# alepnabil/fmcw_radar_processing

Measured on AMD Instinct MI355X. Metric: radar frames/sec (range-FFT+Doppler+STFT) + achieved HBM GB/s vs roofline, higher is better.
Workload: dtype f32

## Files before the change

### fmcw_radar_processing_amd/csrc/fmcw_api.cpp

```cpp
#include "api_internal.h"
#include "xcd_ctr_plan.h"

#include <dlfcn.h>

#include <cmath>
#include <cstdio>
#include <cstring>

namespace {
thread_local std::string g_err;
}

namespace fmcw {

int fail(int code, const std::string& msg) {
  g_err = msg;
  return code;
}

int set_error(int code, const char* msg) { return fail(code, msg); }

void par_memcpy(void* dst, const void* src, size_t n) {
  const unsigned hw = std::max(1u, std::thread::hardware_concurrency());
  const unsigned T = n >= (8u << 20) ? std::min(8u, hw) : 1u;
  if (T == 1) {
    std::memcpy(dst, src, n);
    return;
  }
  const size_t per = ((n + T - 1) / T + 4095) & ~(size_t)4095;
  std::vector<std::thread> th;
  for (unsigned t = 0; t < T; ++t) {
    const size_t o = (size_t)t * per;
    if (o >= n) break;
    th.emplace_back([=] { std::memcpy(static_cast<char*>(dst) + o, static_cast<const char*>(src) + o, std::min(per, n - o)); });
  }
  for (auto& x : th) x.join();
}

const Rccl& rccl() {
  static Rccl r = [] {
    Rccl x;
    void* h = nullptr;
    for (const char* name : {"librccl.so.1", "librccl.so", "/opt/rocm/lib/librccl.so.1"}) {
      h = dlopen(name, RTLD_NOW | RTLD_NOLOAD);
      if (h) break;
    }
    if (!h) h = dlopen("librccl.so.1", RTLD_NOW | RTLD_GLOBAL);
    if (!h) h = dlopen("/opt/rocm/lib/librccl.so.1", RTLD_NOW | RTLD_GLOBAL);
    if (!h) return x;
    x.comm_init_all = reinterpret_cast<decltype(x.comm_init_all)>(dlsym(h, "ncclCommInitAll"));
    x.comm_destroy = reinterpret_cast<decltype(x.comm_destroy)>(dlsym(h, "ncclCommDestroy"));
    x.all_reduce = reinterpret_cast<decltype(x.all_reduce)>(dlsym(h, "ncclAllReduce"));
    x.group_start = reinterpret_cast<decltype(x.group_start)>(dlsym(h, "ncclGroupStart"));
    x.group_end = reinterpret_cast<decltype(x.group_end)>(dlsym(h, "ncclGroupEnd"));
    x.error_string = reinterpret_cast<decltype(x.error_string)>(dlsym(h, "ncclGetErrorString"));
    x.ok = x.comm_init_all && x.comm_destroy && x.all_reduce && x.group_start && x.group_end && x.error_string;
    return x;
  }();
  return r;
}

}

fmcw_ctx::~fmcw_ctx() {
  for (ncclComm_t m : comms) (void)rccl().comm_destroy(m);
  for (fmcw_ctx* q : peers) delete q;
  (void)hipSetDevice(device);
  if (stream) (void)hipStreamSynchronize(stream);
  for (auto& pd : pending) { (void)hipEventDestroy(pd.a); (void)hipEventDestroy(pd.b); }
  for (auto e : pool) (void)hipEventDestroy(e);
  for (int i = 0; i < kSlots; ++i)
    for (hipEvent_t e : {ev_k1[i], ev_k2[i], ev_k3[i]})
      if (e) (void)hipEventDestroy(e);
  for (hipEvent_t e : {ev_fork, ev_join, ev_h2d[0], ev_h2d[1], ev_comp[0], ev_comp[1], ev_d2h[0], ev_d2h[1]})
    if (e) (void)hipEventDestroy(e);
  for (hipStream_t x : {sd, sx, cin, cout})
    if (x) { (void)hipStreamSynchronize(x); (void)hipStreamDestroy(x); }
  if (stream) (void)hipStreamDestroy(stream);
}

float2* fmcw_ctx::stft_tab(hipStream_t st, size_t bytes, int* status) {
  float2* t = static_cast<float2*>(s_tabs.get(st, bytes + STFT_TAPS_BYTES, status));
  if (t) {
    s_tabs.last->key = nullptr;
    s_tabs.last->key_n = 0;
  }
  return t;
}

float2* fmcw_ctx::stft_tab64(hipStream_t st, const float* d_win, int nfft, bool* build, int* status) {
  float2* t = static_cast<float2*>(s_tabs.get(st, (size_t)(nfft / 2 + 1) * 20 * 8 + STFT_TAPS_BYTES, status));
  if (!t) return nullptr;
  PerStream::Entry* e = s_tabs.last;
  *build = !(e->key == d_win && e->key_n == nfft);
  e->key = d_win;
  e->key_n = nfft;
  return t;
}

namespace {

int check_params(const fmcw_params* p) {
  if (!p) return fail(FMCW_E_ARG, "params is NULL");
  if (p->nts < 1 || p->nts > 65536) return fail(FMCW_E_ARG, "nts out of range [1, 65536]");
  if (p->pn < 1 || p->pn > 65536) return fail(FMCW_E_ARG, "pn out of range [1, 65536]");
  if (!fmcw::range_size_supported(p->nr)) return fail(FMCW_E_ARG, "nr must be a power of two in [16, 2048]");
  if (!fmcw::doppler_size_supported(p->nd)) return fail(FMCW_E_ARG, "nd must be a power of two in [2, 1024]");
  if (p->max_targets < 1 || p->max_targets > 8) return fail(FMCW_E_ARG, "max_targets must be in [1, 8]");
  if (!(p->dist_per_bin > 0.f)) return fail(FMCW_E_ARG, "dist_per_bin must be > 0");
  return FMCW_OK;
}

int build_calw(fmcw_ctx* c, float if_scale, hipStream_t s) {
  const size_t n = c->h_wr.size();
  std::vector<float> t(4 * n);
  for (size_t i = 0; i < n; ++i) {
    t[4 * i] = c->h_cal[2 * i];
    t[4 * i + 1] = c->h_cal[2 * i + 1];
    t[4 * i + 2] = (float)((double)if_scale * c->h_wr[i]);
    t[4 * i + 3] = c->h_wr[i];
  }
  CHK(c->calw.ensure(t.size() * 4));
  HIPCHK(hipMemcpyAsync(c->calw.p, t.data(), t.size() * 4, hipMemcpyHostToDevice, s));
  HIPCHK(hipStreamSynchronize(s));
  c->calw_scale = if_scale;
  return FMCW_OK;
}

int check_ctx(fmcw_ctx* c, const fmcw_params* p) {
  if (!c) return fail(FMCW_E_ARG, "ctx is NULL");
  CHK(check_params(p));
  if (!c->taps) return fail(FMCW_E_STATE, "fmcw_set_taps has not been called");
  if (p->nts != c->p.nts || p->pn != c->p.pn || p->nr != c->p.nr || p->nd != c->p.nd)
    return fail(FMCW_E_STATE, "nts/pn/nr/nd differ from the ones given to fmcw_set_taps");
  CHK(set_device(c));
  if (p->if_scale != c->calw_scale) {
    HIPCHK(hipDeviceSynchronize());
    CHK(build_calw(c, p->if_scale, c->stream));
  }
  return FMCW_OK;
}

int upload_twiddles(DevBuf& buf, int n, hipStream_t s) {
  std::vector<float> tw(2 * (size_t)n);
  for (int i = 0; i < n; ++i) {
    const double a = -2.0 * M_PI * (double)i / (double)n;
    tw[2 * i] = (float)std::cos(a);
    tw[2 * i + 1] = (float)std::sin(a);
  }
  CHK(buf.ensure(tw.size() * sizeof(float)));
  HIPCHK(hipMemcpyAsync(buf.p, tw.data(), tw.size() * sizeof(float), hipMemcpyHostToDevice, s));
  HIPCHK(hipStreamSynchronize(s));
  return FMCW_OK;
}

int64_t default_chunk(const fmcw_params* p) {
  const int64_t per_frame = (int64_t)p->pn * p->nr * 8;
  int64_t c = (256ll << 20) / std::max<int64_t>(per_frame, 1);
  return std::max<int64_t>(c, 1);
}

int range_cpt(int nr, int64_t nchirps) {
  const int T = nr >= 16 ? nr / 16 : 1;
  const int teams = T >= 256 ? 1 : 256 / T;
  const int64_t c = nchirps / ((int64_t)teams * 2048);
  return (int)std::max<int64_t>(1, std::min<int64_t>(8, c));
}


}

extern "C" {

int32_t fmcw_abi_version(void) { return FMCW_ABI_VERSION; }

const char* fmcw_last_error(void) { return g_err.c_str(); }

int fmcw_device_count(int32_t* n) {
  if (!n) return fail(FMCW_E_ARG, "n is NULL");
  int d = 0;
  hipError_t e = hipGetDeviceCount(&d);
  if (e != hipSuccess) {
    *n = 0;
    return fail(FMCW_E_HIP, std::string("hipGetDeviceCount: ") + hipGetErrorString(e));
  }
  *n = d;
  return FMCW_OK;
}

int fmcw_default_devices(int32_t cap, int32_t* ids, int32_t* n) {
  if (!ids || !n || cap < 1) return fail(FMCW_E_ARG, "ids/n NULL or cap < 1");
  *n = 0;
  const char* env = std::getenv("FMCW_DEVICES");
  std::string v = env ? env : "";
  v.erase(std::remove_if(v.begin(), v.end(), [](char ch) { return ch == ' ' || ch == '\t'; }), v.end());
  std::vector<long> want;
  if (!v.empty() && v != "all") {
    size_t pos = 0;
    while (pos <= v.size()) {
      const size_t end = std::min(v.find(',', pos), v.size());
      const std::string tok = v.substr(pos, end - pos);
      char* stop = nullptr;
      const long id = tok.empty() ? -1 : std::strtol(tok.c_str(), &stop, 10);
      if (tok.empty() || *stop != '\0' || id < 0) return fail(FMCW_E_ARG, "FMCW_DEVICES: malformed list '" + v + "'");
      want.push_back(id);
      pos = end + 1;
    }
    if ((int64_t)want.size() > cap) return fail(FMCW_E_ARG, "FMCW_DEVICES: more ids than cap");
  }
  int nd = 0;
  hipError_t e = hipGetDeviceCount(&nd);
  if (e != hipSuccess) return fail(FMCW_E_HIP, std::string("hipGetDeviceCount: ") + hipGetErrorString(e));
  if (want.empty()) {
    if (nd < 1) return fail(FMCW_E_HIP, "no HIP device present");
    const int m = std::min<int>(nd, cap);
    for (int i = 0; i < m; ++i) ids[i] = i;
    *n = m;
    return FMCW_OK;
  }
  for (size_t i = 0; i < want.size(); ++i) {
    if (want[i] >= nd)
      return fail(FMCW_E_ARG, "FMCW_DEVICES: device " + std::to_string(want[i]) + " not present (" +
                                  std::to_string(nd) + " devices)");
    ids[i] = (int32_t)want[i];
  }
  *n = (int32_t)want.size();
  return FMCW_OK;
}

static int ctx_create_one(int32_t device_id, fmcw_ctx** out) {
  *out = nullptr;
  int nd = 0;
  HIPCHK(hipGetDeviceCount(&nd));
  if (device_id < 0 || device_id >= nd)
    return fail(FMCW_E_HIP, "device " + std::to_string(device_id) + " not present (" + std::to_string(nd) + " devices)");
  HIPCHK(hipSetDevice(device_id));
  hipDeviceProp_t prop;
  HIPCHK(hipGetDeviceProperties(&prop, device_id));
  if (std::strncmp(prop.gcnArchName, "gfx950", 6) != 0)
    return fail(FMCW_E_HIP, std::string("libfmcw is built for gfx950, device is ") + prop.gcnArchName);
  auto* c = new fmcw_ctx();
  c->device = device_id;
  bool ok = hipStreamCreateWithFlags(&c->stream, hipStreamNonBlocking) == hipSuccess &&
            hipStreamCreateWithFlags(&c->sd, hipStreamNonBlocking) == hipSuccess &&
            hipStreamCreateWithFlags(&c->sx, hipStreamNonBlocking) == hipSuccess &&
            hipStreamCreateWithFlags(&c->cin, hipStreamNonBlocking) == hipSuccess &&
            hipStreamCreateWithFlags(&c->cout, hipStreamNonBlocking) == hipSuccess;
  for (int i = 0; i < 2; ++i)
    for (hipEvent_t* e : {&c->ev_h2d[i], &c->ev_comp[i], &c->ev_d2h[i]})
      ok = ok && hipEventCreateWithFlags(e, hipEventDisableTiming) == hipSuccess;
  for (int i = 0; i < fmcw_ctx::kSlots; ++i)
    for (hipEvent_t* e : {&c->ev_k1[i], &c->ev_k2[i], &c->ev_k3[i]})
      ok = ok && hipEventCreateWithFlags(e, hipEventDisableTiming | fmcw::kEvDevice) == hipSuccess;
  for (hipEvent_t* e : {&c->ev_fork, &c->ev_join})
    ok = ok && hipEventCreateWithFlags(e, hipEventDisableTiming | fmcw::kEvDevice) == hipSuccess;
  if (!ok) {
    delete c;
    return fail(FMCW_E_HIP, "stream/event creation failed");
  }
  *out = c;
  return FMCW_OK;
}

int fmcw_ctx_create(int32_t n_devices, const int32_t* device_ids, fmcw_ctx** out) {
  if (!out) return fail(FMCW_E_ARG, "out is NULL");
  *out = nullptr;
  if (n_devices < 1 || n_devices > 64) return fail(FMCW_E_ARG, "n_devices must be in [1, 64]");
  std::vector<int> ids(n_devices);
  for (int i = 0; i < n_devices; ++i) ids[i] = device_ids ? device_ids[i] : i;
  fmcw_ctx* c = nullptr;
  CHK(ctx_create_one(ids[0], &c));
  for (int i = 1; i < n_devices; ++i) {
    fmcw_ctx* q = nullptr;
    const int st = ctx_create_one(ids[i], &q);
    if (st != FMCW_OK) {
      delete c;
      return st;
    }
    c->peers.push_back(q);
  }
  std::vector<int> sorted = ids;
  std::sort(sorted.begin(), sorted.end());
  const bool distinct = std::adjacent_find(sorted.begin(), sorted.end()) == sorted.end();
  if (n_devices > 1 && distinct) {
    if (!rccl().ok) {
      delete c;
      return fail(FMCW_E_HIP, "RCCL (librccl.so.1) not found: needed for a context over several devices");
    }
    c->comms.assign(n_devices, nullptr);
    const ncclResult_t r = rccl().comm_init_all(c->comms.data(), n_devices, ids.data());
    if (r != ncclSuccess) {
      c->comms.clear();
      const std::string msg = std::string("ncclCommInitAll: ") + rccl().error_string(r);
      delete c;
      return fail(FMCW_E_HIP, msg);
    }
  }
  *out = c;
  return FMCW_OK;
}

int fmcw_ctx_devices(fmcw_ctx* c, int32_t* n_devices, int32_t* device_ids, int32_t* rccl_comms) {
  if (!c || !n_devices) return fail(FMCW_E_ARG, "NULL argument");
  *n_devices = 1 + (int32_t)c->peers.size();
  if (device_ids) {
    device_ids[0] = c->device;
    for (size_t i = 0; i < c->peers.size(); ++i) device_ids[i + 1] = c->peers[i]->device;
  }
  if (rccl_comms) *rccl_comms = c->comms.empty() ? 0 : 1;
  return FMCW_OK;
}

int fmcw_ctx_destroy(fmcw_ctx* c) {
  if (!c) return FMCW_OK;
  delete c;
  return FMCW_OK;
}

int fmcw_set_taps(fmcw_ctx* c, const fmcw_params* p, const float* range_win, const float* doppler_win,
                  const float* calib) {
  if (!c) return fail(FMCW_E_ARG, "ctx is NULL");
  CHK(check_params(p));
  if (!range_win || !doppler_win || !calib) return fail(FMCW_E_ARG, "taps pointer is NULL");
  CHK(set_device(c));
  hipStream_t s = c->stream;
  HIPCHK(hipDeviceSynchronize());
  CHK(c->wd.ensure((size_t)p->pn * 4));
  CHK(c->cal.ensure((size_t)p->nts * 8));
  HIPCHK(hipMemcpyAsync(c->wd.p, doppler_win, (size_t)p->pn * 4, hipMemcpyHostToDevice, s));
  HIPCHK(hipMemcpyAsync(c->cal.p, calib, (size_t)p->nts * 8, hipMemcpyHostToDevice, s));
  c->h_wr.assign(range_win, range_win + p->nts);
  c->h_cal.assign(calib, calib + 2 * (size_t)p->nts);
  double sr = 0, si = 0;
  for (int n = 0; n < p->nts; ++n) { sr += calib[2 * n]; si += calib[2 * n + 1]; }
  c->cal_sum = make_float2((float)sr, (float)si);
  CHK(build_calw(c, p->if_scale, s));
  CHK(upload_twiddles(c->tw_nr, p->nr, s));
  CHK(upload_twiddles(c->tw_nd, p->nd, s));
  c->p = *p;
  c->taps = true;
  c->x_tab_ok = false;
  HIPCHK(hipStreamSynchronize(s));
  for (fmcw_ctx* q : c->peers) CHK(fmcw_set_taps(q, p, range_win, doppler_win, calib));
  return FMCW_OK;
}

int fmcw_set_chunk_frames(fmcw_ctx* c, int64_t frames) {
  if (!c) return fail(FMCW_E_ARG, "ctx is NULL");
  if (frames < 0) return fail(FMCW_E_ARG, "frames < 0");
  c->chunk_frames = frames;
  for (fmcw_ctx* q : c->peers) q->chunk_frames = frames;
  return FMCW_OK;
}

int fmcw_set_pipeline(fmcw_ctx* c, int32_t mode) {
  if (!c) return fail(FMCW_E_ARG, "ctx is NULL");
  if (mode != FMCW_PIPE_AUTO && mode != FMCW_PIPE_STREAMS && mode != FMCW_PIPE_ONEPASS && mode != FMCW_PIPE_XCD)
    return fail(FMCW_E_ARG, "bad pipeline mode");
  c->pipe_mode = mode;
  for (fmcw_ctx* q : c->peers) q->pipe_mode = mode;
  return FMCW_OK;
}

static int xcd_check(fmcw_ctx* c) {
  if (!c->xcd_used) return FMCW_OK;
  unsigned e = 0;
  HIPCHK(hipMemcpy(&e, c->x_err.p, sizeof(e), hipMemcpyDeviceToHost));
  c->xcd_used = false;
  if (!e) return FMCW_OK;
  HIPCHK(hipMemset(c->x_err.p, 0, sizeof(e)));
  return fail(FMCW_E_HIP, (e & 2) ? "XCD schedule: an XCD received more than 32 workgroups (outputs invalid)"
                                  : "XCD schedule: a range-cube hand-off timed out (outputs invalid)");
}

int fmcw_rdx_clock(fmcw_ctx* c, double* mhz, double* us) {
  if (!c || !mhz) return fail(FMCW_E_ARG, "ctx / mhz is NULL");
  *mhz = 0.0;
  if (us) *us = 0.0;
  CHK(set_device(c));
  if (!c->x_clk.p) return FMCW_OK;
  unsigned long long h[4] = {};
  HIPCHK(hipStreamSynchronize(c->stream));
  HIPCHK(hipDeviceSynchronize());
  HIPCHK(hipMemcpy(h, c->x_clk.p, sizeof(h), hipMemcpyDeviceToHost));
  if (h[3] > h[1] && h[2] > h[0]) {
    *mhz = (double)(h[2] - h[0]) / (double)(h[3] - h[1]) * 100.0;
    if (us) *us = (double)(h[3] - h[1]) / 100.0;
  }
  return FMCW_OK;
}

int fmcw_copy_device(fmcw_ctx* c, const void* d_src, void* d_dst, int64_t bytes, void* stream) {
  if (!c) return fail(FMCW_E_ARG, "ctx is NULL");
  if (!d_src || !d_dst || bytes < 0) return fail(FMCW_E_ARG, "bad copy arguments");
  CHK(set_device(c));
  HIPCHK(fmcw::launch_copy16(d_src, d_dst, bytes, pick(c, stream)));
  return FMCW_OK;
}

int fmcw_synchronize(fmcw_ctx* c) {
  if (!c) return fail(FMCW_E_ARG, "ctx is NULL");
  CHK(set_device(c));
  HIPCHK(hipStreamSynchronize(c->stream));
  return xcd_check(c);
}

int fmcw_timing_enable(fmcw_ctx* c, int32_t enable) {
  if (!c) return fail(FMCW_E_ARG, "ctx is NULL");
  if (enable < 0 || enable > 3) return fail(FMCW_E_ARG, "timing level must be 0, 1, 2 or 3");
  c->timing = enable;
  return FMCW_OK;
}

static int timing_collect(fmcw_ctx* c) {
  for (auto& pd : c->pending) {
    HIPCHK(hipEventSynchronize(pd.b));
    float ms = 0.f;
    HIPCHK(hipEventElapsedTime(&ms, pd.a, pd.b));
    c->total_ms[pd.stage] += ms;
    c->launches[pd.stage] += 1;
    c->pool.push_back(pd.a);
    c->pool.push_back(pd.b);
  }
  c->pending.clear();
  return FMCW_OK;
}

int fmcw_timing_read(fmcw_ctx* c, int32_t stage, double* total_ms, int64_t* launches) {
  if (!c) return fail(FMCW_E_ARG, "ctx is NULL");
  if (stage < 0 || stage >= kStages) return fail(FMCW_E_ARG, "stage out of range");
  CHK(set_device(c));
  CHK(timing_collect(c));
  if (total_ms) *total_ms = c->total_ms[stage];
  if (launches) *launches = c->launches[stage];
  return FMCW_OK;
}

int fmcw_timing_reset(fmcw_ctx* c) {
  if (!c) return fail(FMCW_E_ARG, "ctx is NULL");
  CHK(set_device(c));
  CHK(timing_collect(c));
  for (int i = 0; i < kStages; ++i) { c->total_ms[i] = 0; c->launches[i] = 0; }
  return FMCW_OK;
}

static int build_xcd_tab(fmcw_ctx* c, hipStream_t s) {
  const int NR = c->p.nr;
  std::vector<double> cr(NR), ci(NR);
  for (int i = 0; i < NR; ++i) {
    const double a = -2.0 * M_PI * (double)i / (double)NR;
    cr[i] = std::cos(a);
    ci[i] = std::sin(a);
  }
  std::vector<float> xt(2 * (size_t)fmcw::XT_SIZE);
  auto xput = [&](int idx, int e1024) { xt[2 * idx] = (float)cr[e1024 & (NR - 1)]; xt[2 * idx + 1] = (float)ci[e1024 & (NR - 1)]; };
  for (int l = 0; l < 64; ++l) {
    for (int k1 = 1; k1 < 8; ++k1)
      for (int e = 0; e < 2; ++e) xput(fmcw::XT_R1 + (2 * (k1 - 1) + e) * 64 + l, (2 * l + e) * k1);
    for (int s1 = 1; s1 < 16; ++s1) xput(fmcw::XT_R2 + (s1 - 1) * 64 + l, 8 * ((l & 7) * s1));
    for (int d0 = 1; d0 < 16; ++d0) xput(fmcw::XT_D1 + (d0 - 1) * 64 + l, 4 * ((l & 15) * d0));
    for (int k1 = 1; k1 < 8; ++k1) xput(fmcw::XT_H1 + (k1 - 1) * 64 + l, 2 * l * k1);
    for (int s1 = 1; s1 < 8; ++s1) xput(fmcw::XT_H2 + (s1 - 1) * 64 + l, 16 * ((l & 7) * s1));
    for (int s2 = 0; s2 < 8; ++s2) xput(fmcw::XT_HC + s2 * 64 + l, l + 64 * s2);
  }
  CHK(c->x_tab.ensure(xt.size() * 4));
  HIPCHK(hipMemcpyAsync(c->x_tab.p, xt.data(), xt.size() * 4, hipMemcpyHostToDevice, s));
  HIPCHK(hipStreamSynchronize(s));
  c->x_tab_ok = true;
  return FMCW_OK;
}

static unsigned host_s16mask(const fmcw_params* p, int NR) {
  {
    const char* e = std::getenv("FMCW_S16");
    if (e && e[0] == '0') return 0u;
  }
  const double dpb = p->dist_per_bin;
  if (!(dpb > 0.0) || !std::isfinite(dpb) || !std::isfinite(p->min_d) || !std::isfinite(p->max_d)) return 0u;
  const double lo_d = std::floor((double)p->min_d / dpb) - 2, hi_d = std::ceil((double)p->max_d / dpb) + 2;
  const int lo = (int)std::max(0.0, std::min((double)NR, lo_d));
  const int hi = (int)std::max(-1.0, std::min((double)NR - 1, hi_d));
  unsigned m = 0;
  for (int b = 0; b < NR / 128; ++b)
    if (hi < lo || 128 * b + 127 < lo || 128 * b > hi) m |= 1u << b;
  return m;
}

struct SlowLeg {
  int32_t* list;
  int64_t* len;
  float* pmax;
};

static int process_onepass(fmcw_ctx* c, const fmcw_params* p, const void* d_iq, int h, int64_t F, float* d_prof,
                           int32_t* d_count, int32_t* d_ridx, float* d_rmag, int32_t* d_didx, float* d_slow,
                           void* d_rd, int64_t probe_column, float* d_probe, const SlowLeg* leg, hipStream_t s) {
  const int C = p->pn, S = p->nts, NR = p->nr, ND = p->nd, M = p->max_targets;
  const int64_t chunk = std::min<int64_t>(F, c->chunk_frames > 0 ? c->chunk_frames : 8192);
  const int tiles = fmcw::XCD_TILES, ncand = fmcw::XCD_CAND;
  const int TC = tiles * ncand;
  const int slots = fmcw::XCD_MAX_SLOTS;
  {
#ifdef FMCW_XCUBE_PAD_AB
    CHK(c->x_cube.ensure((size_t)8 * slots * fmcw::XCD_TILES * C * 32 * 8 + ((size_t)1 << 30)));
#else
    CHK(c->x_cube.ensure((size_t)8 * slots * fmcw::XCD_TILES * C * 32 * 8));
#endif
    if (!c->x_ctr.p) {
      CHK(c->x_ctr.ensure(sizeof(unsigned) * 2 * fmcw::XCD_CTR_WORDS));
      HIPCHK(hipMemsetAsync(c->x_ctr.p, 0, sizeof(unsigned) * 2 * fmcw::XCD_CTR_WORDS, s));
      c->x_ctr_set = 0;
    }
    if (!c->x_clk.p) {
      CHK(c->x_clk.ensure(4 * sizeof(unsigned long long)));
      HIPCHK(hipMemsetAsync(c->x_clk.p, 0, 4 * sizeof(unsigned long long), s));
    }
    if (!c->x_err.p) {
      CHK(c->x_err.ensure(sizeof(unsigned)));
      HIPCHK(hipMemsetAsync(c->x_err.p, 0, sizeof(unsigned), s));
    }
  }
  CHK(c->op_rowpk.ensure((size_t)chunk * NR * 8));
  CHK(c->op_cidx.ensure((size_t)chunk * TC * 4));
  CHK(c->op_crows.ensure((size_t)chunk * TC * C * 4));
  int32_t* det_done = nullptr;
  if (leg) {
    int st = FMCW_OK;
    bool fresh = false;
    det_done = static_cast<int32_t*>(c->det_done.get(s, 9 * 128, &st, &fresh));
    CHK(st);
    if (fresh) HIPCHK(hipMemsetAsync(det_done, 0, 9 * 128, s));
  }
  const int64_t pframe = probe_column > 0 ? (probe_column - 1) / C : -1;
  const int pchirp = probe_column > 0 ? (int)((probe_column - 1) % C) : 0;
  if (!c->x_tab_ok) CHK(build_xcd_tab(c, s));
  if (pframe >= 0 && d_probe) {
    fmcw::ProbeArgs pa{};
    pa.iq = d_iq; pa.h = h;
    pa.frame = pframe; pa.chirp = pchirp; pa.C = C; pa.S = S; pa.NR = NR;
    pa.calw = c->calw.as<float4>(); pa.tw_nr = c->tw_nr.as<float2>(); pa.probe_mag = d_probe;
    HIPCHK(fmcw::launch_probe(pa, s));
  }
  StageTimer span(c, 7, s, 1);
  for (int64_t f0 = 0; f0 < F; f0 += chunk) {
    const int64_t nf = std::min(chunk, F - f0);
    fmcw::OnePassArgs a{};
    a.iq = static_cast<const char*>(d_iq) + (size_t)f0 * C * S * (h ? 4 : 8);
    a.h = h;
    a.rd_scale = h ? 1.0f / ((float)NR * ND) : 1.0f;
    a.F = nf; a.C = C; a.S = S;
    a.calw = c->calw.as<float4>();
    a.tw_nr = c->tw_nr.as<float2>(); a.tw_nd = c->tw_nd.as<float2>(); a.wd = c->wd.as<float>();
    a.rd = d_rd ? static_cast<char*>(d_rd) + (size_t)f0 * NR * ND * (h ? 4 : 8) : nullptr;
    a.profile = d_prof + f0 * NR;
    a.rowpk = c->op_rowpk.as<int2>();
    a.cand_idx = c->op_cidx.as<int32_t>();
    a.cand_rows = c->op_crows.as<float>();
    a.range_thr = p->range_thr; a.min_d = p->min_d; a.max_d = p->max_d; a.dist_per_bin = p->dist_per_bin;
    const bool xmemset = [] { const char* e = std::getenv("FMCW_XCD_MEMSET"); return e && e[0] == '1'; }();
    const fmcw::XcdCtrPlan xp = fmcw::xcd_ctr_plan(c->x_ctr_set, xmemset);
    a.xcube = c->x_cube.as<float2>(); a.xerr = c->x_err.as<unsigned>();
    a.xctr = c->x_ctr.as<unsigned>() + xp.count_set * fmcw::XCD_CTR_WORDS;
    a.xclr = xp.clear_set < 0 ? nullptr : c->x_ctr.as<unsigned>() + xp.clear_set * fmcw::XCD_CTR_WORDS;
    a.xmemset = xp.memset_first ? 1 : 0;
#ifdef FMCW_XCUBE_PAD_AB
    if (const char* e = std::getenv("FMCW_XCUBE_PAD")) {
      const size_t pad = std::min<size_t>((size_t)std::strtoull(e, nullptr, 0), (size_t)1 << 30) & ~(size_t)255;
      a.xcube = reinterpret_cast<float2*>(c->x_cube.as<char>() + pad);
    }
#endif
    a.slots = slots; a.xtab = c->x_tab.as<float2>(); a.cal_sum = c->cal_sum;
    a.clk = c->x_clk.as<unsigned long long>();
    a.s16mask = h ? host_s16mask(p, NR) : 0u;
    a.nteams = c->xcd_teams > 0 ? c->xcd_teams : 0;
    std::memcpy(a.xcc_team, c->xcc_team, sizeof(a.xcc_team));
    {
      const char* e = std::getenv("FMCW_ONEPASS_FORCE_FIX");
      a.force_fix = (e && e[0] == '1') ? 1 : 0;
    }
#if defined(XK_STAMPS) || defined(XK_SKEW)
    static unsigned long long* xdbg = nullptr;
    if (!xdbg) HIPCHK(hipMalloc(&xdbg, (size_t)1 << 20));
    a.dbg = xdbg;
#endif
    {
      StageTimer tm(c, 8, s, 2);
      {
        HIPCHK(fmcw::launch_xcd(a, s));
        c->xcd_used = true;
        if (nf > 0) c->x_ctr_set = xp.next_set;
#ifdef XK_SKEW
        {
          constexpr int ST = 256;
          const int nblk = 32 * a.nteams;
          std::vector<unsigned long long> hh((size_t)nblk * 2 * ST);
          HIPCHK(hipStreamSynchronize(s));
          HIPCHK(hipMemcpy(hh.data(), a.dbg, hh.size() * 8, hipMemcpyDeviceToHost));
          double spread = 0, lag_min = 0, lag_max = 0, lag_mean = 0, pub_to_first_poll = 0;
          long n = 0;
          std::vector<long> last(32, 0), first(32, 0);
          for (int xx = 0; xx < a.nteams; ++xx)
            for (int j = 8; j < ST - 8; ++j) {
              unsigned long long pmin = ~0ull, pmax = 0, qmin = ~0ull, qmax = 0;
              double qs = 0;
              int kl = 0, kf = 0;
              for (int kk = 0; kk < 32; ++kk) {
                const unsigned long long p_ = hh[((size_t)(xx * 32 + kk)) * 2 * ST + 2 * j];
                const unsigned long long q_ = hh[((size_t)(xx * 32 + kk)) * 2 * ST + 2 * j + 1];
                if (p_ > pmax) { pmax = p_; kl = kk; }
                if (p_ < pmin) { pmin = p_; kf = kk; }
                qmin = std::min(qmin, q_); qmax = std::max(qmax, q_);
                qs += (double)q_;
              }
              if (!pmin || !qmin) continue;
              spread += (double)(pmax - pmin);
              lag_min += (double)qmin - (double)pmax;
              lag_max += (double)qmax - (double)pmax;
              lag_mean += qs / 32 - (double)pmax;
              pub_to_first_poll += (double)qmin - (double)pmin;
              ++last[kl]; ++first[kf]; ++n;
            }
          if (n) {
            std::fprintf(stderr, "xk-skew (us, %ld team-steps): publish spread %.2f | poll return after the last publish: "
                         "first %.2f mean %.2f last %.2f\n", n, spread / n / 100, lag_min / n / 100, lag_mean / n / 100,
                         lag_max / n / 100);
            std::fprintf(stderr, "xk-skew last publisher by member:");
            for (int kk = 0; kk < 32; ++kk) std::fprintf(stderr, " %ld", last[kk]);
            std::fprintf(stderr, "\nxk-skew first publisher by member:");
            for (int kk = 0; kk < 32; ++kk) std::fprintf(stderr, " %ld", first[kk]);
            std::fprintf(stderr, "\n");
          }
        }
#endif
#ifdef XK_STAMPS
        {
          const int nblk = 32 * a.nteams;
          std::vector<unsigned long long> hh(nblk * 32);
          HIPCHK(hipStreamSynchronize(s));
          HIPCHK(hipMemcpy(hh.data(), a.dbg, hh.size() * 8, hipMemcpyDeviceToHost));
          static const char* nm[10] = {"B1", "stage", "B2", "rows", "pubwait+B3", "cand", "R1+ld+D3",
                                       "poll+grp", "TD..R3", "RD"};
          for (int wv = 0; wv < 2; ++wv) {
            double ph[10] = {}, steps = 0;
            for (int bb = 0; bb < nblk; ++bb) {
              for (int q = 0; q < 10; ++q) ph[q] += (double)hh[(bb * 2 + wv) * 16 + q];
              steps += (double)hh[(bb * 2 + wv) * 16 + 15];
            }
            double tot = 0;
            std::fprintf(stderr, "xk-stamps wave %d (us/step):", wv * 4);
            for (int q = 0; q < 10; ++q) { std::fprintf(stderr, " %s %.2f |", nm[q], ph[q] / steps / 100); tot += ph[q]; }
            double cyc = 0, rt = 0;
            for (int bb = 0; bb < nblk; ++bb) { cyc += (double)hh[(bb * 2 + wv) * 16 + 13]; rt += (double)hh[(bb * 2 + wv) * 16 + 14]; }
            std::fprintf(stderr, " sum %.2f | clock %.3f GHz\n", tot / steps / 100, rt > 0 ? cyc / rt * 0.1 : 0.0);
          }
        }
#endif
      }
      tm.done();
    }
    fmcw::Detect1pArgs k{};
    k.profile = a.profile; k.rowpk = a.rowpk; k.rd = a.rd; k.ND = ND; k.rd_h = h; k.cand_idx = a.cand_idx; k.cand_rows = a.cand_rows;
    k.tiles = tiles; k.ncand = ncand;
    k.nframes = (int)nf; k.NR = NR; k.C = C; k.M = M;
    k.det.ND = ND; k.det.C = C; k.det.M = M;
    k.det.range_thr = p->range_thr; k.det.doppler_thr = p->doppler_thr;
    k.det.min_d = p->min_d; k.det.max_d = p->max_d; k.det.dist_per_bin = p->dist_per_bin;
    k.det.fallback = p->doppler_fallback_idx;
    k.det.cube_unscale = 1.0f; k.det.rd_unscale = 1.0f / a.rd_scale;
    k.count = d_count + f0; k.ridx = d_ridx + f0 * M; k.rmag = d_rmag + f0 * M; k.didx = d_didx + f0 * M;
    k.slow_mag = d_slow + f0 * C;
    k.iq = a.iq; k.h = h; k.S = S; k.calw = a.calw; k.tw_nr = a.tw_nr;
    if (leg && f0 + nf == F) {
      k.done = det_done; k.count_all = d_count; k.F_all = F; k.pn = C;
      k.list = leg->list; k.len = leg->len; k.pmax_reset = leg->pmax;
    }
    {
      StageTimer tm(c, 2, s, 2);
      HIPCHK(fmcw::launch_detect_1p(k, s));
      tm.done();
    }
  }
  if (leg) CHK(c->det_done.done(s));
  span.done();
  return FMCW_OK;
}

static int process_device_impl(fmcw_ctx* c, const fmcw_params* p, const void* d_iq, int32_t in_dtype, int64_t F,
                               float* d_prof, int32_t* d_count, int32_t* d_ridx, float* d_rmag, int32_t* d_didx,
                               float* d_slow, void* d_cube, void* d_rd, int32_t out_dtype, int64_t probe_column,
                               float* d_probe, const SlowLeg* leg, void* stream) {
  CHK(check_ctx(c, p));
  if (F < 0) return fail(FMCW_E_ARG, "F < 0");
  if (F == 0) return FMCW_OK;
  if (in_dtype != FMCW_C64 && in_dtype != FMCW_C32H) return fail(FMCW_E_ARG, "bad in_dtype");
  if (out_dtype != FMCW_C64 && out_dtype != FMCW_C32H) return fail(FMCW_E_ARG, "bad out_dtype");
  if (!d_iq || !d_prof || !d_count || !d_ridx || !d_rmag || !d_didx || !d_slow)
    return fail(FMCW_E_ARG, "required device pointer is NULL");
  const int S = p->nts, C = p->pn, NR = p->nr, ND = p->nd, M = p->max_targets;
  if (probe_column < 0 || probe_column > F * (int64_t)C) return fail(FMCW_E_ARG, "probe_column out of range");
  hipStream_t s = pick(c, stream);
  const bool onepass_ok = !d_cube && (!d_rd || out_dtype == in_dtype) && fmcw::onepass_supported(S, C, NR, ND);
  const bool want = c->pipe_mode == FMCW_PIPE_ONEPASS || c->pipe_mode == FMCW_PIPE_XCD;
  if (want || (c->pipe_mode == FMCW_PIPE_AUTO && onepass_ok)) {
    if (!onepass_ok)
      return fail(FMCW_E_ARG, "single-pass schedule: needs nr 1024, pn == nd == 256, even nts <= nr, "
                              "the RD map in the IQ dtype and no range cube");
    if (c->xcd_teams < 0) {
      int n = 0;
      HIPCHK(fmcw::xcd_census(&n, c->xcc_team));
      const char* e = std::getenv("FMCW_NO_XCD");
      c->xcd_teams = (e && e[0] == '1') ? 0 : n;
    }
    if (c->xcd_teams > 0)
      return process_onepass(c, p, d_iq, in_dtype == FMCW_C32H ? 1 : 0, F, d_prof, d_count, d_ridx, d_rmag, d_didx,
                             d_slow, d_rd, probe_column, d_probe, leg, s);
    if (want)
      return fail(FMCW_E_ARG, "XCD schedule: needs 32 CUs per XCD and a grid of one workgroup per CU dealt 32 per XCD");
  }
  const int64_t chunk = c->chunk_frames > 0 ? c->chunk_frames : default_chunk(p);
  const int cube_dt = d_cube ? out_dtype : FMCW_C64;
  const int rd_dt = d_rd ? out_dtype : FMCW_C64;
  const float cube_scale = cube_dt == FMCW_C32H ? 1.0f / NR : 1.0f;
  const float rd_scale = rd_dt == FMCW_C32H ? 1.0f / ((float)NR * ND) : 1.0f;
  const int64_t cf = std::min(chunk, F);
  const size_t cube_slot = (size_t)cf * C * NR * 8, rd_slot = (size_t)cf * NR * ND * 8;
  constexpr int NS = fmcw_ctx::kSlots;
  if (!d_cube) CHK(c->scratch_cube.ensure(NS * cube_slot));
  if (!d_rd) CHK(c->scratch_rd.ensure(NS * rd_slot));
  const int64_t pframe = probe_column > 0 ? (probe_column - 1) / C : -1;
  const int pchirp = probe_column > 0 ? (int)((probe_column - 1) % C) : 0;
  hipStream_t sd = c->sd, sx = c->sx;
  if (F <= chunk) sd = sx = s;
  if (const char* e = std::getenv("FMCW_ONE_STREAM"); e && e[0] == '1') sd = sx = s;
  const bool split = sd != s || sx != s;
  StageTimer span(c, 7, s, 1);
  if (split) {
    HIPCHK(hipEventRecord(c->ev_fork, s));
    HIPCHK(hipStreamWaitEvent(sd, c->ev_fork, 0));
    HIPCHK(hipStreamWaitEvent(sx, c->ev_fork, 0));
  }

  int64_t i = 0;
  for (int64_t f0 = 0; f0 < F; f0 += chunk, ++i) {
    const int b = (int)(i % NS);
    const int64_t nf = std::min(chunk, F - f0);
    if (split && i >= NS) HIPCHK(hipStreamWaitEvent(s, c->ev_k3[b], 0));
    char* cube = d_cube ? static_cast<char*>(d_cube) + (size_t)f0 * C * NR * esize(cube_dt)
                        : c->scratch_cube.as<char>() + b * cube_slot;
    char* rd = d_rd ? static_cast<char*>(d_rd) + (size_t)f0 * NR * ND * esize(rd_dt)
                    : c->scratch_rd.as<char>() + b * rd_slot;

    fmcw::RangeArgs ra{};
    ra.iq = static_cast<const char*>(d_iq) + (size_t)f0 * C * S * esize(in_dtype);
    ra.in_dtype = in_dtype;
    ra.nchirps = nf * C;
    ra.C = C; ra.S = S; ra.NR = NR;
    ra.calw = c->calw.as<float4>();
    ra.cal_sum = c->cal_sum;
    ra.if_scale = p->if_scale;
    ra.tw = c->tw_nr.as<float2>();
    ra.cube = cube;
    ra.cube_dtype = cube_dt;
    ra.cube_scale = cube_scale;
    ra.profile = nullptr;
    ra.cpt = range_cpt(NR, ra.nchirps);
    {
      StageTimer tm(c, 0, s, 2);
      HIPCHK(fmcw::launch_range(ra, s));
      tm.done();
    }
    if (split) {
      HIPCHK(hipEventRecord(c->ev_k1[b], s));
      HIPCHK(hipStreamWaitEvent(sd, c->ev_k1[b], 0));
    }

    fmcw::DopplerArgs da{};
    da.cube = cube; da.cube_dtype = cube_dt;
    da.cube_unscale = 1.0f / cube_scale; da.rd_scale = rd_scale;
    da.nframes = (int)nf; da.C = C; da.NR = NR; da.ND = ND;
    da.wd = c->wd.as<float>();
    da.tw = c->tw_nd.as<float2>();
    da.rd = rd; da.rd_dtype = rd_dt;
    da.profile = d_prof + f0 * NR;
    {
      StageTimer tm(c, 1, sd, 2);
      HIPCHK(fmcw::launch_doppler(da, sd));
      tm.done();
    }
    if (split) {
      HIPCHK(hipEventRecord(c->ev_k2[b], sd));
      HIPCHK(hipStreamWaitEvent(sx, c->ev_k2[b], 0));
    }

    fmcw::DetectArgs ka{};
    ka.profile = d_prof + f0 * NR;
    ka.rd = rd; ka.rd_dtype = rd_dt;
    ka.cube = cube; ka.cube_dtype = cube_dt;
    ka.cube_unscale = 1.0f / cube_scale; ka.rd_unscale = 1.0f / rd_scale;
    ka.nframes = (int)nf; ka.NR = NR; ka.ND = ND; ka.C = C; ka.M = M;
    ka.range_thr = p->range_thr; ka.doppler_thr = p->doppler_thr;
    ka.min_d = p->min_d; ka.max_d = p->max_d; ka.dist_per_bin = p->dist_per_bin;
    ka.fallback = p->doppler_fallback_idx;
    ka.count = d_count + f0;
    ka.ridx = d_ridx + f0 * M;
    ka.rmag = d_rmag + f0 * M;
    ka.didx = d_didx + f0 * M;
    ka.slow_mag = d_slow + f0 * C;
    ka.probe_frame = (pframe >= f0 && pframe < f0 + nf) ? pframe - f0 : -1;
    ka.probe_chirp = pchirp;
    ka.probe_mag = d_probe;
    {
      StageTimer tm(c, 2, sx, 2);
      HIPCHK(fmcw::launch_detect(ka, sx));
      tm.done();
    }
    if (split) HIPCHK(hipEventRecord(c->ev_k3[b], sx));
  }
  span.s = sd;
  span.done();
  if (split) {
    HIPCHK(hipEventRecord(c->ev_join, sx));
    HIPCHK(hipStreamWaitEvent(s, c->ev_join, 0));
  }
  if (leg) {
    HIPCHK(fmcw::launch_compact(d_count, F, C, leg->list, leg->len, s));
    if (leg->pmax) HIPCHK(hipMemsetAsync(leg->pmax, 0, 4, s));
  }
  return FMCW_OK;
}

int fmcw_process_device(fmcw_ctx* c, const fmcw_params* p, const void* d_iq, int32_t in_dtype, int64_t F,
                        float* d_prof, int32_t* d_count, int32_t* d_ridx, float* d_rmag, int32_t* d_didx,
                        float* d_slow, void* d_cube, void* d_rd, int32_t out_dtype, int64_t probe_column,
                        float* d_probe, void* stream) {
  return process_device_impl(c, p, d_iq, in_dtype, F, d_prof, d_count, d_ridx, d_rmag, d_didx, d_slow, d_cube, d_rd,
                             out_dtype, probe_column, d_probe, nullptr, stream);
}

int fmcw_process_slow_device(fmcw_ctx* c, const fmcw_params* p, const void* d_iq, int32_t in_dtype, int64_t F,
                             float* d_prof, int32_t* d_count, int32_t* d_ridx, float* d_rmag, int32_t* d_didx,
                             float* d_slow, void* d_rd, int32_t out_dtype, int32_t* d_frame_list, int64_t* d_len,
                             float* d_pmax, void* stream) {
  if (!d_frame_list || !d_len) return fail(FMCW_E_ARG, "d_frame_list / d_len is NULL");
  if (F == 0 && c) {
    CHK(check_ctx(c, p));
    hipStream_t s = pick(c, stream);
    HIPCHK(hipMemsetAsync(d_len, 0, 8, s));
    if (d_pmax) HIPCHK(hipMemsetAsync(d_pmax, 0, 4, s));
    return FMCW_OK;
  }
  const SlowLeg leg{d_frame_list, d_len, d_pmax};
  return process_device_impl(c, p, d_iq, in_dtype, F, d_prof, d_count, d_ridx, d_rmag, d_didx, d_slow, nullptr, d_rd,
                             out_dtype, 0, nullptr, &leg, stream);
}

int fmcw_range_fft_device(fmcw_ctx* c, const fmcw_params* p, const void* d_iq, int32_t in_dtype, int64_t F,
                          void* d_cube, int32_t out_dtype, float* d_prof, void* stream) {
  CHK(check_ctx(c, p));
  if (F < 0) return fail(FMCW_E_ARG, "F < 0");
  if (F == 0) return FMCW_OK;
  if (!d_iq || !d_cube || !d_prof) return fail(FMCW_E_ARG, "required device pointer is NULL");
  if (in_dtype != FMCW_C64 && in_dtype != FMCW_C32H) return fail(FMCW_E_ARG, "bad in_dtype");
  if (out_dtype != FMCW_C64 && out_dtype != FMCW_C32H) return fail(FMCW_E_ARG, "bad out_dtype");
  hipStream_t s = pick(c, stream);
  HIPCHK(hipMemsetAsync(d_prof, 0, (size_t)F * p->nr * 4, s));
  fmcw::RangeArgs ra{};
  ra.iq = d_iq; ra.in_dtype = in_dtype;
  ra.nchirps = F * p->pn;
  ra.C = p->pn; ra.S = p->nts; ra.NR = p->nr;
  ra.calw = c->calw.as<float4>(); ra.cal_sum = c->cal_sum; ra.if_scale = p->if_scale;
  ra.tw = c->tw_nr.as<float2>();
  ra.cube = d_cube; ra.cube_dtype = out_dtype;
  ra.cube_scale = out_dtype == FMCW_C32H ? 1.0f / p->nr : 1.0f;
  ra.profile = d_prof;
  int cpt = 8;
  if (const char* e = std::getenv("FMCW_K1_CPT")) cpt = std::max(1, std::min(64, std::atoi(e)));
  while (cpt > 1 && (p->pn % cpt) != 0) cpt >>= 1;
  ra.cpt = cpt;
  const int T = p->nr >= 16 ? p->nr / 16 : 1;
  const int teams = T >= 256 ? 1 : 256 / T;
  const int64_t per_wg = (int64_t)teams * cpt;
  ra.parts = (per_wg < p->pn && p->pn % per_wg == 0) ? (int)(p->pn / per_wg) : 0;
  if (ra.parts > 1) {
    int st = FMCW_OK;
    ra.prof_part = static_cast<float*>(c->k1_part.get(s, (size_t)F * ra.parts * p->nr * 4, &st));
    CHK(st);
  }
  StageTimer tm(c, 6, s);
  HIPCHK(fmcw::launch_range(ra, s));
  if (ra.parts > 1) {
    HIPCHK(fmcw::launch_profile_reduce(ra.prof_part, ra.parts, F, p->nr, d_prof, s));
    CHK(c->k1_part.done(s));
  }
  tm.done();
  return FMCW_OK;
}

int fmcw_compact_device(fmcw_ctx* c, const int32_t* d_count, int64_t F, int32_t pn, int32_t* d_list,
                        int64_t* d_len, void* stream) {
  if (!c) return fail(FMCW_E_ARG, "ctx is NULL");
  if (F < 0 || pn < 1) return fail(FMCW_E_ARG, "bad F / pn");
  if (!d_count || !d_list || !d_len) return fail(FMCW_E_ARG, "NULL device pointer");
  CHK(set_device(c));
  hipStream_t s = pick(c, stream);
  StageTimer tm(c, 3, s);
  HIPCHK(fmcw::launch_compact(d_count, F, pn, d_list, d_len, s));
  tm.done();
  return FMCW_OK;
}

}

struct BigOut {
  char* host;
  size_t fbytes;
};
template <typename Run>
static int host_pipeline(fmcw_ctx* c, const void* iq, int64_t F, size_t fin, const BigOut (&big)[2], Run&& run) {
  hipStream_t s = c->stream;
  const int64_t Fc = host_chunk(fin, F);
  const size_t slot_in = (size_t)Fc * fin;
  size_t slot_big[2], off_big[2] = {0, 0}, slot_out = 0;
  bool any = false;
  for (int q = 0; q < 2; ++q) {
    slot_big[q] = big[q].host ? (size_t)Fc * big[q].fbytes : 0;
    off_big[q] = slot_out;
    slot_out += slot_big[q];
    any = any || big[q].host;
  }
  CHK(c->h_iq.ensure(2 * slot_in));
  CHK(c->pin_in.ensure(2 * slot_in));
  if (any) {
    CHK(c->h_rd.ensure(2 * slot_out));
    CHK(c->pin_out.ensure(2 * slot_out));
  }
  const int64_t n = (F + Fc - 1) / Fc;
  auto drain = [&](int64_t j) -> int {
    const int b = (int)(j & 1);
    const int64_t f0 = j * Fc, nf = std::min(Fc, F - f0);
    HIPCHK(hipEventSynchronize(c->ev_d2h[b]));
    for (int q = 0; q < 2; ++q)
      if (big[q].host)
        par_memcpy(big[q].host + (size_t)f0 * big[q].fbytes, c->pin_out.at(b * slot_out + off_big[q]),
                   (size_t)nf * big[q].fbytes);
    return FMCW_OK;
  };
  const bool single = n == 1;
  hipStream_t cin = single ? s : c->cin;
  if (!single) {
    HIPCHK(hipEventRecord(c->ev_fork, s));
    HIPCHK(hipStreamWaitEvent(c->cin, c->ev_fork, 0));
  }
  for (int64_t i = 0; i < n; ++i) {
    const int b = (int)(i & 1);
    const int64_t f0 = i * Fc, nf = std::min(Fc, F - f0);
    if (i >= 2) HIPCHK(hipEventSynchronize(c->ev_h2d[b]));
    par_memcpy(c->pin_in.at(b * slot_in), static_cast<const char*>(iq) + (size_t)f0 * fin, (size_t)nf * fin);
    if (i >= 2) HIPCHK(hipStreamWaitEvent(c->cin, c->ev_comp[b], 0));
    HIPCHK(hipMemcpyAsync(c->h_iq.as<char>() + b * slot_in, c->pin_in.at(b * slot_in), (size_t)nf * fin,
                          hipMemcpyHostToDevice, cin));
    if (!single) {
      HIPCHK(hipEventRecord(c->ev_h2d[b], c->cin));
      HIPCHK(hipStreamWaitEvent(s, c->ev_h2d[b], 0));
    }
    if (any && i >= 2) {
      HIPCHK(hipStreamWaitEvent(s, c->ev_d2h[b], 0));
      CHK(drain(i - 2));
    }
    char* d_big[2];
    for (int q = 0; q < 2; ++q) d_big[q] = big[q].host ? c->h_rd.as<char>() + b * slot_out + off_big[q] : nullptr;
    CHK(run(c->h_iq.as<char>() + b * slot_in, f0, nf, d_big));
    HIPCHK(hipEventRecord(c->ev_comp[b], s));
    if (any) {
      HIPCHK(hipStreamWaitEvent(c->cout, c->ev_comp[b], 0));
      for (int q = 0; q < 2; ++q)
        if (big[q].host)
          HIPCHK(hipMemcpyAsync(c->pin_out.at(b * slot_out + off_big[q]), d_big[q], (size_t)nf * big[q].fbytes,
                                hipMemcpyDeviceToHost, c->cout));
      HIPCHK(hipEventRecord(c->ev_d2h[b], c->cout));
    }
  }
  if (any)
    for (int64_t j = std::max<int64_t>(0, n - 2); j < n; ++j) CHK(drain(j));
  return FMCW_OK;
}

extern "C" {

static int process_host_one(fmcw_ctx* c, const fmcw_params* p, const void* iq, int32_t in_dtype, int64_t F,
                            float* prof, int32_t* count, int32_t* ridx, float* rmag, int32_t* didx, float* slow,
                            float* cube, float* rd, int64_t probe_column, float* probe) {
  CHK(check_ctx(c, p));
  if (F < 0) return fail(FMCW_E_ARG, "F < 0");
  if (F == 0) return FMCW_OK;
  if (!iq || !prof || !count || !ridx || !rmag || !didx || !slow) return fail(FMCW_E_ARG, "required pointer is NULL");
  if (in_dtype != FMCW_C64 && in_dtype != FMCW_C32H) return fail(FMCW_E_ARG, "bad in_dtype");
  const int S = p->nts, C = p->pn, NR = p->nr, ND = p->nd, M = p->max_targets;
  hipStream_t s = c->stream;
  Arena ar;
  const size_t o_prof = ar.add((size_t)F * NR * 4), o_count = ar.add((size_t)F * 4), o_ridx = ar.add((size_t)F * M * 4),
               o_rmag = ar.add((size_t)F * M * 4), o_didx = ar.add((size_t)F * M * 4), o_slow = ar.add((size_t)F * C * 4),
               o_probe = ar.add(probe ? (size_t)NR * 4 : 0);
  CHK(c->h_small.ensure(ar.off));
  CHK(c->pin_small.ensure(ar.off));
  char* const hs = c->h_small.as<char>();
  auto at = [&](size_t o) { return reinterpret_cast<float*>(hs + o); };
  auto ati = [&](size_t o) { return reinterpret_cast<int32_t*>(hs + o); };
  const size_t fin = (size_t)C * S * esize(in_dtype);
  const BigOut big[2] = {{reinterpret_cast<char*>(cube), (size_t)C * NR * 8}, {reinterpret_cast<char*>(rd), (size_t)NR * ND * 8}};
  CHK(host_pipeline(c, iq, F, fin, big, [&](char* d_in, int64_t f0, int64_t nf, char* const* d_big) {
    const int64_t pc = probe && probe_column > f0 * C && probe_column <= (f0 + nf) * C ? probe_column - f0 * C : 0;
    return fmcw_process_device(c, p, d_in, in_dtype, nf, at(o_prof) + f0 * NR, ati(o_count) + f0, ati(o_ridx) + f0 * M,
                               at(o_rmag) + f0 * M, ati(o_didx) + f0 * M, at(o_slow) + f0 * C, d_big[0], d_big[1], FMCW_C64,
                               pc, pc ? at(o_probe) : nullptr, s);
  }));
  HIPCHK(hipMemcpyAsync(c->pin_small.p, hs, ar.off, hipMemcpyDeviceToHost, s));
  HIPCHK(hipStreamSynchronize(s));
  HIPCHK(hipStreamSynchronize(c->cout));
  const char* ps = c->pin_small.at(0);
  par_memcpy(prof, ps + o_prof, (size_t)F * NR * 4);
  std::memcpy(count, ps + o_count, (size_t)F * 4);
  std::memcpy(ridx, ps + o_ridx, (size_t)F * M * 4);
  std::memcpy(rmag, ps + o_rmag, (size_t)F * M * 4);
  std::memcpy(didx, ps + o_didx, (size_t)F * M * 4);
  par_memcpy(slow, ps + o_slow, (size_t)F * C * 4);
  if (probe) std::memcpy(probe, ps + o_probe, (size_t)NR * 4);
  return xcd_check(c);
}

static int range_fft_host_one(fmcw_ctx* c, const fmcw_params* p, const void* iq, int32_t in_dtype, int64_t F,
                              float* cube, float* prof) {
  CHK(check_ctx(c, p));
  if (F < 0) return fail(FMCW_E_ARG, "F < 0");
  if (F == 0) return FMCW_OK;
  if (!iq || !cube || !prof) return fail(FMCW_E_ARG, "required pointer is NULL");
  if (in_dtype != FMCW_C64 && in_dtype != FMCW_C32H) return fail(FMCW_E_ARG, "bad in_dtype");
  const int S = p->nts, C = p->pn, NR = p->nr;
  hipStream_t s = c->stream;
  CHK(c->h_prof.ensure((size_t)F * NR * 4));
  const BigOut big[2] = {{reinterpret_cast<char*>(cube), (size_t)C * NR * 8}, {nullptr, 0}};
  CHK(host_pipeline(c, iq, F, (size_t)C * S * esize(in_dtype), big, [&](char* d_in, int64_t f0, int64_t nf, char* const* d_big) {
    return fmcw_range_fft_device(c, p, d_in, in_dtype, nf, d_big[0], FMCW_C64, c->h_prof.as<float>() + f0 * NR, s);
  }));
  HIPCHK(hipMemcpyAsync(prof, c->h_prof.p, (size_t)F * NR * 4, hipMemcpyDeviceToHost, s));
  HIPCHK(hipStreamSynchronize(s));
  HIPCHK(hipStreamSynchronize(c->cout));
  return FMCW_OK;
}

}

extern "C" {

int fmcw_process(fmcw_ctx* c, const fmcw_params* p, const void* iq, int32_t in_dtype, int64_t F, float* prof,
                 int32_t* count, int32_t* ridx, float* rmag, int32_t* didx, float* slow, float* cube, float* rd,
                 int64_t probe_column, float* probe) {
  CHK(check_ctx(c, p));
  if (F < 0) return fail(FMCW_E_ARG, "F < 0");
  if (in_dtype != FMCW_C64 && in_dtype != FMCW_C32H) return fail(FMCW_E_ARG, "bad in_dtype");
  if (probe_column < 0 || probe_column > F * (int64_t)p->pn) return fail(FMCW_E_ARG, "probe_column out of range");
  const int C = p->pn, S = p->nts, NR = p->nr, ND = p->nd, M = p->max_targets;
  const size_t fin = (size_t)C * S * esize(in_dtype);
  return over_devices(c, F, [&](fmcw_ctx* d, int, int64_t f0, int64_t n) {
    const int64_t pc = probe_column > f0 * C && probe_column <= (f0 + n) * C ? probe_column - f0 * C : 0;
    return process_host_one(d, p, static_cast<const char*>(iq) + f0 * fin, in_dtype, n, prof + f0 * NR, count + f0,
                            ridx + f0 * M, rmag + f0 * M, didx + f0 * M, slow + f0 * C,
                            cube ? cube + f0 * (size_t)C * NR * 2 : nullptr, rd ? rd + f0 * (size_t)NR * ND * 2 : nullptr,
                            pc, pc ? probe : nullptr);
  });
}

int fmcw_range_fft(fmcw_ctx* c, const fmcw_params* p, const void* iq, int32_t in_dtype, int64_t F, float* cube,
                   float* prof) {
  CHK(check_ctx(c, p));
  if (F < 0) return fail(FMCW_E_ARG, "F < 0");
  if (in_dtype != FMCW_C64 && in_dtype != FMCW_C32H) return fail(FMCW_E_ARG, "bad in_dtype");
  const size_t fin = (size_t)p->pn * p->nts * esize(in_dtype);
  return over_devices(c, F, [&](fmcw_ctx* d, int, int64_t f0, int64_t n) {
    return range_fft_host_one(d, p, static_cast<const char*>(iq) + f0 * fin, in_dtype, n,
                              cube + f0 * (size_t)p->pn * p->nr * 2, prof + f0 * p->nr);
  });
}

int fmcw_synth_device(fmcw_ctx* c, const fmcw_params* p, int64_t frame0, int64_t F, void* d_iq, int32_t dtype,
                      void* stream) {
  CHK(check_ctx(c, p));
  if (F < 0 || frame0 < 0) return fail(FMCW_E_ARG, "F / frame0 < 0");
  if (!d_iq) return fail(FMCW_E_ARG, "d_iq is NULL");
  if (dtype != FMCW_C64 && dtype != FMCW_C32H) return fail(FMCW_E_ARG, "bad dtype");
  fmcw::SynthArgs a{};
  a.iq = d_iq; a.dtype = dtype; a.frame0 = frame0; a.nframes = F;
  a.C = p->pn; a.S = p->nts; a.NR = p->nr; a.ND = p->nd;
  a.dist_per_bin = p->dist_per_bin;
  a.cal = c->cal.as<float2>();
  HIPCHK(fmcw::launch_synth(a, pick(c, stream)));
  return FMCW_OK;
}

}
```

### fmcw_radar_processing_amd/csrc/fmcw_internal.h

```cpp
#pragma once
#include <hip/hip_runtime.h>
#include <stdint.h>

namespace fmcw {

#ifndef FMCW_EV_SYSFENCE
constexpr unsigned kEvDevice = hipEventDisableSystemFence;
#else
constexpr unsigned kEvDevice = 0;
#endif

struct RangeArgs {
  const void* iq;
  int in_dtype;
  int64_t nchirps;
  int C, S, NR;
  const float4* calw;
  float2 cal_sum;
  float if_scale;
  const float2* tw;
  void* cube;
  int cube_dtype;
  float cube_scale;
  float* profile;
  int cpt;
  float* prof_part;
  int parts;
};

struct DopplerArgs {
  const void* cube;
  int cube_dtype;
  float cube_unscale;
  float rd_scale;
  int nframes, C, NR, ND;
  const float* wd;
  const float2* tw;
  void* rd;
  int rd_dtype;
  float* profile;
};

struct DetectArgs {
  const float* profile;
  const void* rd;
  int rd_dtype;
  const void* cube;
  int cube_dtype;
  float cube_unscale, rd_unscale;
  int nframes, NR, ND, C, M;
  float range_thr, doppler_thr, min_d, max_d, dist_per_bin;
  int fallback;
  int32_t* count;
  int32_t* ridx;
  float* rmag;
  int32_t* didx;
  float* slow_mag;
  int64_t probe_frame;
  int probe_chirp;
  float* probe_mag;
};

struct DetectParams {
  int ND, C, M;
  float range_thr, doppler_thr, min_d, max_d, dist_per_bin;
  int fallback;
  float cube_unscale, rd_unscale;
};

struct OnePassArgs {
  const void* iq;
  int h;
  float rd_scale;
  int64_t F;
  int C, S;
  const float4* calw;
  const float2* tw_nr;
  const float2* tw_nd;
  const float* wd;
  void* rd;
  float* profile;
  int2* rowpk;
  int32_t* cand_idx;
  float* cand_rows;
  float range_thr, min_d, max_d, dist_per_bin;
  int force_fix;
  unsigned long long* dbg;
  unsigned long long* clk;
  float2* xcube;
  unsigned* xctr;
  unsigned* xclr;
  unsigned* xerr;
  int slots;
  unsigned s16mask;
  int nteams;
  int xmemset;
  int8_t xcc_team[16];
  const float2* xtab;
  float2 cal_sum;
};

constexpr int XCD_TILES = 32;
constexpr int XCD_CAND = 2;
constexpr int XCD_MAX_SLOTS = 4;
constexpr int XCD_GRID = 256;
constexpr int XCD_TICKETS = 8 * 2 * 32 * XCD_MAX_SLOTS;
constexpr int XCD_ABORT = XCD_TICKETS + 8 * 32;
constexpr int XCD_IDLE = XCD_ABORT + 32;
constexpr int XCD_CTR_WORDS = XCD_IDLE + 256 * 32;
constexpr int XT_R1 = 0;
constexpr int XT_R2 = 14 * 64;
constexpr int XT_D1 = 29 * 64;
constexpr int XT_H1 = 44 * 64;
constexpr int XT_H2 = 51 * 64;
constexpr int XT_HC = 58 * 64;
constexpr int XT_SIZE = 66 * 64;
#ifndef XK_HALF
__host__ __device__ inline int xcd_bin(int g, int p) {
  return (p >> 3) + 4 * (g & 1) + 8 * ((g >> 1) & 1) + 16 * (p & 7) + 128 * (g >> 2);
}
__host__ __device__ inline int xcd_group(int r) { return ((r >> 2) & 1) | (((r >> 3) & 1) << 1) | ((r >> 7) << 2); }
__host__ __device__ inline int xcd_pos(int r) { return ((r & 3) << 3) | ((r >> 4) & 7); }
#else
__host__ __device__ inline int xcd_bin(int g, int p) { return 32 * g + p; }
__host__ __device__ inline int xcd_group(int r) { return r >> 5; }
__host__ __device__ inline int xcd_pos(int r) { return r & 31; }
#endif

struct Detect1pArgs {
  const float* profile;
  const int2* rowpk;
  const void* rd;
  int ND, rd_h;
  const int32_t* cand_idx;
  const float* cand_rows;
  int tiles, ncand;
  int nframes, NR, C, M;
  DetectParams det;
  int32_t* count;
  int32_t* ridx;
  float* rmag;
  int32_t* didx;
  float* slow_mag;
  const void* iq;
  int h, S;
  const float4* calw;
  const float2* tw_nr;
  int32_t* done;
  const int32_t* count_all;
  int64_t F_all;
  int pn;
  int32_t* list;
  int64_t* len;
  float* pmax_reset;
};

hipError_t launch_detect_1p(const Detect1pArgs& a, hipStream_t s);
hipError_t launch_xcd(const OnePassArgs& a, hipStream_t s);
hipError_t xcd_census(int* nteams, int8_t* xcc_team);

struct ProbeArgs {
  const void* iq;
  int h;
  int64_t frame;
  int chirp, C, S, NR;
  const float4* calw;
  const float2* tw_nr;
  float* probe_mag;
};
hipError_t launch_probe(const ProbeArgs& a, hipStream_t s);
bool onepass_supported(int nts, int pn, int nr, int nd);

struct StftArgs {
  const float* slow_mag;
  const int32_t* frame_list;
  const int64_t* len;
  int pn;
  const float* halo;
  int n_halo;
  const int64_t* halo_len;
  const float* win;
  int wlen, hop, nfft;
  float inv_fs;
  int64_t max_seg;
  float* P;
  float* pmax;
  int64_t* nseg_out;
  const int32_t* bins;
  int ncol;
  const int32_t* tiles;
  int ntiles;
  int table_form;
};

bool stft_fast_path(int wlen, int hop);
bool stft64_form(int nfft);
enum StftForm { STFT_FORM_TABLE = 0, STFT_FORM_64F = 1, STFT_FORM_64M = 2 };
StftForm stft_form(const StftArgs& a, int mode, const float* dst);
hipError_t launch_stft_table(const float* win, int nfft, float2* tab, hipStream_t s);
hipError_t launch_stft20(const StftArgs& a, const float2* tab, int mode, float* dst, hipStream_t s, int64_t dst_cap,
                         int64_t tab_cap);


struct StftDbArgs {
  const float* P;
  const int64_t* nseg;
  int64_t max_seg;
  int nbins_in;
  const float* pmax;
  int nlog;
  const int32_t* lidx;
  const float* lw;
  float* out;
};

struct SynthArgs {
  void* iq;
  int dtype;
  int64_t frame0, nframes;
  int C, S, NR, ND;
  float dist_per_bin;
  const float2* cal;
};

hipError_t launch_range(const RangeArgs& a, hipStream_t s);
hipError_t launch_profile_reduce(const float* part, int parts, int64_t frames, int nr, float* profile, hipStream_t s);
hipError_t launch_doppler(const DopplerArgs& a, hipStream_t s);
hipError_t launch_detect(const DetectArgs& a, hipStream_t s);
hipError_t launch_compact(const int32_t* count, int64_t F, int pn, int32_t* frame_list, int64_t* len,
                          hipStream_t s);
hipError_t launch_stft_power(const StftArgs& a, hipStream_t s);
hipError_t launch_stft_db(const StftDbArgs& a, hipStream_t s);
hipError_t launch_synth(const SynthArgs& a, hipStream_t s);
hipError_t launch_fill_u32(uint32_t* p, uint32_t v, int64_t n, hipStream_t s);
hipError_t launch_copy16(const void* src, void* dst, int64_t bytes, hipStream_t s);


struct CfarArgs {
  const void* rd;
  int h;
  float scale;
  int64_t F;
  int NR, ND;
  int gr, gd, tr, td;
  int g0, g1;
  int K, local_max;
  float alpha;
  int RS, strips;
  int TC, tiles, waves;
  int32_t* sub_count;
  float4* sub_list;
  int32_t* det_count;
  int32_t* det_ridx;
  int32_t* det_didx;
  float* det_power;
  float* det_noise;
  uint8_t* mask;
};
void cfar_plan(CfarArgs& a, int64_t F);
size_t cfar_scratch_per_frame(const CfarArgs& a);
hipError_t launch_cfar(const CfarArgs& a, hipStream_t s);

struct SigArgs {
  const void* rd;
  int h;
  float scale2;
  int64_t F;
  int NR, ND;
  int g0, g1;
  int th;
  int dc;
  const int32_t* center;
  int64_t cstride;
  int SR, slabs;
  float* part;
  float* dt;
  float* rt;
  float* dt_max;
  float* rt_max;
};
void sig_plan(SigArgs& a);
size_t sig_scratch_per_frame(const SigArgs& a);
hipError_t launch_sig(const SigArgs& a, hipStream_t s);
hipError_t launch_sig_db(const float* map, int64_t n, const float* mx, float floor_db, float* out, hipStream_t s);

struct ClusterArgs {
  int64_t F;
  int ND;
  int K;
  int link_r, link_d, min_cells, max_tgt;
  const int32_t* det_count;
  const int32_t* det_ridx;
  const int32_t* det_didx;
  const float* det_power;
  const float* det_noise;
  int32_t* tgt_count;
  int32_t* cells; int32_t* pk_ridx; int32_t* pk_didx; int32_t* ext_r; int32_t* ext_d;
  float* pk_power; float* pk_noise; float* power; float* range; float* doppler;
  int32_t* det_label;
};
hipError_t launch_cluster(const ClusterArgs& a, hipStream_t s);

constexpr int kAoaChan = 8;
struct AoaArgs {
  int64_t F;
  int NR, ND;
  int K;
  int A;
  int M;
  int h;
  int tgt_any;
  float scale2;
  float kinv;
  float w[2 * kAoaChan];
  const void* rd[kAoaChan];
  const int32_t* det_count;
  const int32_t* det_ridx;
  const int32_t* det_didx;
  const int32_t* det_label;
  float* det_zre; float* det_zim; float* det_phase; float* det_sin;
  float* tgt_zre; float* tgt_zim; float* tgt_e0; float* tgt_e1; float* tgt_phase; float* tgt_sin; float* tgt_coh;
  int32_t* tgt_cells;
};
hipError_t launch_aoa(const AoaArgs& a, hipStream_t s);

constexpr int kTrackFields = 9;
constexpr int kTrackMax = 64;
constexpr int track_state_words(int max_trk) { return (kTrackFields * max_trk + 1 + 3) & ~3; }
struct TrackArgs {
  int64_t S, F;
  int NR, ND;
  int M, T;
  float wr, wd;
  float alpha_r, alpha_d, beta_r;
  int confirm_hits, max_coast;
  const int32_t* tgt_count;
  const float* range;
  const float* doppler;
  const float* power;
  uint32_t* state;
  int32_t* trk_count;
  int32_t* trk_id; int32_t* trk_status; int32_t* trk_age; int32_t* trk_misses;
  float* trk_range; float* trk_rate; float* trk_doppler; float* trk_power;
  int32_t* tgt_track;
};
hipError_t launch_track(const TrackArgs& a, hipStream_t s);

constexpr int kMtiRingC64 = 4;
constexpr int kMtiRingC32H = 8;
struct MtiArgs {
  const void* rd;
  void* out;
  float* bg;
  int32_t* seen;
  int64_t S, F;
  int64_t n16;
  int bpf;
  int h;
  int ring;
  float lambda;
  int ramp, freeze;
};
bool mti_ring_ok(int ring);
hipError_t launch_mti(const MtiArgs& a, hipStream_t s);

bool range_size_supported(int nr);
bool doppler_size_supported(int nd);

struct RenderArgs {
  const float* Q;
  int nq;
  const int64_t* nseg;
  const float* pmax;
  int nb, nfft, seam;
  double fs, t0, dt;
  double fmax, cmin, cmax;
  int W, H;
  uint8_t* img;
};
hipError_t launch_render(const RenderArgs& a, hipStream_t s);

}

#include "host_io.h"
```

### fmcw_radar_processing_amd/csrc/kernels_xcd.hip

```cpp
#include "op_math.h"

#include <cstdio>
#include <cstdlib>
#include <mutex>

namespace fmcw {
namespace xk {
using namespace op;

#ifdef XK_NOREF
#define XK_REF 0
#else
#define XK_REF 1
#endif
#ifndef XK_RD_AUX
#define XK_RD_AUX 2
#endif
constexpr int kRdAux = XK_RD_AUX;
#ifndef XK_LAG
#define XK_LAG 1
#endif
#ifndef XK_NS
#define XK_NS (2 * XK_LAG)
#endif
constexpr int kLag = XK_LAG;
#ifndef XK_POLLAT
#define XK_POLLAT 2
#endif
#ifndef XK_SKEW_STEPS
#define XK_SKEW_STEPS 256
#endif
static_assert(kLag == 1 || kLag == 2, "poll lag 1 (shipped) or 2");
constexpr int kNS = XK_NS;
static_assert(kNS >= 2 * kLag && kNS <= 4, "slot reuse: seeing ready(j - lag) proves frame j - 2 lag read");
constexpr int NK = 32;
constexpr int C = 256;
constexpr int NW = 8;
constexpr int GP = 32;
typedef unsigned u2v __attribute__((ext_vector_type(2)));
typedef unsigned u4v __attribute__((ext_vector_type(4)));
static_assert(NK * NW == C && NK * GP == NR && NK == XCD_TILES, "team geometry");

struct LdsX {
  union {
    f4v stg[C * 17];
    c2 rt[NW][1216];
  } u;
#ifndef XK_HALF
  f4v tw1[7][64];
  f4v tw2[8][64];
#else
  c2 th1[7][64];
  c2 th2[7][64];
  c2 thc[8][64];
#endif
  f4v twd[8][64];
  f4v wdl[4][64];
  f4v wq[4][64];
  c2 cwq[16][64];
  float key[GP];
#ifndef XK_NOREF
#ifndef XK_HALF
  f4v x0[512];
#else
  f4v x0[2][512];
  c2 psum[8];
#endif
#endif
};

__device__ __forceinline__ unsigned ld_flag(const unsigned* p) {
  const unsigned long long u = reinterpret_cast<unsigned long long>(p);
  const unsigned long long su = ((unsigned long long)__builtin_amdgcn_readfirstlane((unsigned)(u >> 32)) << 32) |
                                (unsigned)__builtin_amdgcn_readfirstlane((unsigned)u);
  unsigned v;
  asm volatile("s_load_dword %0, %1, 0x0 glc\n\ts_waitcnt lgkmcnt(0)" : "=s"(v) : "s"(reinterpret_cast<const unsigned*>(su)) : "memory");
  return v;
}
__device__ __forceinline__ void wait_ge(const unsigned* p, unsigned v, unsigned* abort, unsigned* err) {
  for (int it = 0; it < (1 << 20); ++it) {
    if (ld_flag(p) >= v) return;
    if ((it & 63) == 63 && ld_flag(abort)) return;
#ifndef XK_PSLEEP
#define XK_PSLEEP 2
#endif
    __builtin_amdgcn_s_sleep(XK_PSLEEP);
  }
  if (threadIdx.x == 0) {
    typedef __attribute__((address_space(1))) unsigned gu32;
    __hip_atomic_fetch_or((gu32*)abort, 1u, __ATOMIC_RELAXED, __HIP_MEMORY_SCOPE_AGENT);
    __hip_atomic_fetch_or((gu32*)err, 1u, __ATOMIC_RELAXED, __HIP_MEMORY_SCOPE_AGENT);
  }
}
__device__ __forceinline__ void cfence() { asm volatile("" ::: "memory"); }
__device__ __forceinline__ float2 h2f(unsigned b) {
  __half2 h;
  __builtin_memcpy(&h, &b, 4);
  return __half22float2(h);
}

template <int N> __device__ __forceinline__ void vm_wait() {
  static_assert(N >= 0 && N < 64, "vmcnt is 6 bits");
  asm volatile("s_waitcnt vmcnt(%0)" ::"n"(N) : "memory");
}


__device__ __forceinline__ float row_sum16(float v) {
  v += dppf<0xB1>(v);
  v += dppf<0x4E>(v);
  v += dppf<0x141>(v);
  return v + dppf<0x140>(v);
}
__device__ __forceinline__ int row_max16(int v) {
  v = max(v, dppi<0xB1>(v));
  v = max(v, dppi<0x4E>(v));
  v = max(v, dppi<0x141>(v));
  return max(v, dppi<0x140>(v));
}
__device__ __forceinline__ int row_min16(int v) {
  v = min(v, dppi<0xB1>(v));
  v = min(v, dppi<0x4E>(v));
  v = min(v, dppi<0x141>(v));
  return min(v, dppi<0x140>(v));
}

__device__ __forceinline__ f4v pair_cols(c2 A, c2 B, bool odd) {
  const c2 snd = odd ? A : B;
  const c2 rcv = c2{dppf<0xB1>(snd.x), dppf<0xB1>(snd.y)};
  return odd ? f4v{rcv.x, rcv.y, B.x, B.y} : f4v{A.x, A.y, rcv.x, rcv.y};
}

}

template <bool FULL, bool H, bool RD>
__global__ __launch_bounds__(512, 1) void k_rdx(OnePassArgs a) {
  using namespace xk;
  __shared__ __attribute__((aligned(16))) LdsX L;
  const int tid = threadIdx.x, lane = tid & 63;
  const int w = __builtin_amdgcn_readfirstlane(tid >> 6);
  __shared__ int team[2];
  __shared__ unsigned gflag;
  if (tid == 0) {
    gflag = 0;
    unsigned xcc;
    asm volatile("s_getreg_b32 %0, hwreg(HW_REG_XCC_ID)" : "=s"(xcc));
    const int xx = a.xcc_team[xcc & 15];
    int kk = NK;
    if (xx >= 0) kk = (int)__hip_atomic_fetch_add(a.xctr + XCD_TICKETS + xx * 32, 1u, __ATOMIC_RELAXED, __HIP_MEMORY_SCOPE_AGENT);
    if (kk >= NK) { atomicOr(a.xerr, 2u); atomicOr(a.xctr + XCD_ABORT, 1u); }
    team[0] = xx;
    team[1] = kk;
  }
  __syncthreads();
  if (a.xclr && blockIdx.x == 0)
    for (int i = tid; i < XCD_IDLE; i += 512) a.xclr[i] = 0u;
  const int x = __builtin_amdgcn_readfirstlane(team[0]), k = __builtin_amdgcn_readfirstlane(team[1]);
  if (k >= NK) return;
  const bool stamper = a.clk != nullptr && x == 0 && k == 0 && tid == 0;
  if (stamper) {
    a.clk[0] = __builtin_amdgcn_s_memtime();
    a.clk[1] = __builtin_amdgcn_s_memrealtime();
  }
  const int T = a.nteams;
  const int nj = a.F > x ? (int)((a.F - x + T - 1) / T) : 0;
  const int S = FULL ? NR : a.S, S2 = S >> 1, NS = a.slots;
  unsigned* ready = a.xctr + (x * 2 + 0) * 32 * XCD_MAX_SLOTS;
  auto rdy = [&](int s_) __attribute__((always_inline)) -> unsigned* { return &ready[s_ * 32]; };
#ifdef XK_DONE
  unsigned* done = ready + 32 * XCD_MAX_SLOTS;
#endif

  using TP = std::conditional_t<H, h4v, f4v>;
  const TP* __restrict__ iq = reinterpret_cast<const TP*>(a.iq);
  constexpr int kES = 8;
  constexpr int64_t kSlotBytes = (int64_t)NK * C * GP * kES;
  const unsigned s16m = H ? a.s16mask : 0u;
  const bool g16 = (s16m >> (k >> 2)) & 1;
  constexpr float kXS = 1.0f / NR, kXU = (float)NR;
#ifndef XK_NOREF
  TP x0n{};
  auto ld_ref = [&](int64_t f) __attribute__((always_inline)) {
    const TP* __restrict__ q = iq + f * C * (int64_t)S2;
    if constexpr (FULL) x0n = __builtin_nontemporal_load(q + tid);
    else x0n = __builtin_nontemporal_load(q + (tid < S2 ? tid : 0));
  };
  auto put_ref = [&](int b) __attribute__((always_inline)) {
    f4v t;
    if constexpr (H) t = __builtin_convertvector(x0n, f4v);
    else t = x0n;
    if constexpr (!FULL)
      if (tid >= S2) t = f4v{0.f, 0.f, 0.f, 0.f};
#ifndef XK_HALF
    (void)b;
    L.x0[tid] = t;
#else
    L.x0[b][tid] = t;
#endif
  };
  if (nj > 0) ld_ref(x);
#endif
#ifndef XK_HALF
  for (int i = tid; i < 44 * 64; i += 512) {
    const c2 v = tov(a.xtab[i]);
    const int l = i & 63;
    c2* d;
    if (i < XT_R2) { const int t = i >> 6; d = reinterpret_cast<c2*>(&L.tw1[t >> 1][l]) + (t & 1); }
    else if (i < XT_D1) { const int t = (i - XT_R2) >> 6; d = reinterpret_cast<c2*>(&L.tw2[t >> 1][l]) + (t & 1); }
    else { const int t = (i - XT_D1) >> 6; d = reinterpret_cast<c2*>(&L.twd[t >> 1][l]) + (t & 1); }
    *d = v;
  }
#else
  for (int i = XT_D1 + tid; i < XT_H1; i += 512) {
    const int t = (i - XT_D1) >> 6;
    reinterpret_cast<c2*>(&L.twd[t >> 1][i & 63])[t & 1] = tov(a.xtab[i]);
  }
  for (int i = tid; i < 22 * 64; i += 512) {
    const c2 v = tov(a.xtab[XT_H1 + i]);
    const int t = i >> 6, l = i & 63;
    if (t < 7) L.th1[t][l] = v;
    else if (t < 14) L.th2[t - 7][l] = v;
    else L.thc[t - 14][l] = v;
  }
#endif
  const float wd_scale = (H && RD ? a.rd_scale : 1.0f) * (g16 ? kXU : 1.0f);
  for (int i = tid; i < 16 * 64; i += 512)
    reinterpret_cast<float*>(&L.wdl[i >> 8][i & 63])[(i >> 6) & 3] = a.wd[(i & 15) + 16 * (i >> 6)] * wd_scale;
  for (int i = tid; i < 16 * 64; i += 512) {
    const int l = i & 63, v = i >> 6, n = 2 * l + (v & 1) + 128 * (v >> 1);
    const float4 cv = n < S ? a.calw[n] : make_float4(0.f, 0.f, 0.f, 0.f);
    reinterpret_cast<float*>(&L.wq[v >> 2][l])[v & 3] = cv.z;
    L.cwq[v][l] = c2{cv.x * cv.z, cv.y * cv.z};
  }
  const c2 csum = c2{a.cal_sum.x, a.cal_sum.y};
  const float invS = 1.0f / (float)S;
#ifndef XK_NOREF
  if (nj > 0) put_ref(0);
#endif
  __syncthreads();
#ifdef XK_PRIO
  if (w >= 4) __builtin_amdgcn_s_setprio(1);
#endif
#ifdef XK_STAMPS
  constexpr int NST = 10;
  unsigned long long st_acc[NST] = {}, st_t = __builtin_amdgcn_s_memrealtime();
  const unsigned long long st_c0 = __builtin_amdgcn_s_memtime(), st_r0 = st_t;
  auto stamp = [&](int i) {
    const unsigned long long n = __builtin_amdgcn_s_memrealtime();
    st_acc[i] += n - st_t;
    st_t = n;
  };
#else
  auto stamp = [](int) {};
#endif


  auto ld_chirp = [&](int64_t f, TP (&xin)[8]) __attribute__((always_inline)) {
    const TP* __restrict__ q = iq + (f * C + (k * NW + w)) * (int64_t)S2;
#pragma unroll
    for (int i = 0; i < 8; ++i) {
      const int p = lane + 64 * i;
      if constexpr (FULL) xin[i] = __builtin_nontemporal_load(q + p);
      else xin[i] = __builtin_nontemporal_load(q + (p < S2 ? p : 0));
    }
  };

  c2* const rt = L.u.rt[w];
#ifndef XK_HALF
#ifndef XK_NOREF
  const bool refw = k == 0 && w == 0;
  const float dsc = refw ? 0.f : 1.f;
  const c2 csum_w = refw ? csum : c2{0.f, 0.f};
#endif
  auto r_prep = [&](const TP (&xin)[8], c2 (&z0)[8], c2 (&z1)[8]) __attribute__((always_inline)) {
    c2 v[16];
#pragma unroll
    for (int i = 0; i < 8; ++i) {
      f4v t;
      if constexpr (H) t = __builtin_convertvector(xin[i], f4v);
      else t = xin[i];
#ifndef XK_NOREF
      t = __builtin_elementwise_fma(f4v{-dsc, -dsc, -dsc, -dsc}, L.x0[lane + 64 * i], t);
#endif
      if constexpr (!FULL)
        if (!(lane + 64 * i < S2)) t = f4v{0.f, 0.f, 0.f, 0.f};
      v[2 * i] = t.xy;
      v[2 * i + 1] = t.zw;
    }
    c2 sm = (v[0] + v[1]) + (v[2] + v[3]);
#pragma unroll
    for (int n = 4; n < 16; n += 4) sm += (v[n] + v[n + 1]) + (v[n + 2] + v[n + 3]);
    float wv[16];
#pragma unroll
    for (int g = 0; g < 4; ++g) {
      const f4v t = L.wq[g][lane];
      wv[4 * g] = t.x; wv[4 * g + 1] = t.y; wv[4 * g + 2] = t.z; wv[4 * g + 3] = t.w;
    }
#ifndef XK_NOREF
    const c2 mu = (wave_sum_c(sm) - csum_w) * invS;
    if (refw) {
#pragma unroll
      for (int n = 0; n < 16; ++n) v[n] = __builtin_elementwise_fma(v[n] - mu, c2{wv[n], wv[n]}, -L.cwq[n][lane]);
    } else {
#pragma unroll
      for (int n = 0; n < 16; ++n) v[n] = (v[n] - mu) * wv[n];
    }
#else
    const c2 mu = (wave_sum_c(sm) - csum) * invS;
#pragma unroll
    for (int n = 0; n < 16; ++n) v[n] = __builtin_elementwise_fma(v[n] - mu, c2{wv[n], wv[n]}, -L.cwq[n][lane]);
#endif
#pragma unroll
    for (int i = 0; i < 8; ++i) { z0[i] = v[2 * i]; z1[i] = v[2 * i + 1]; }
#ifndef XK_NORANGEFFT
    dft8p(z0);
    dft8p(z1);
#pragma unroll
    for (int k1 = 1; k1 < 8; ++k1) {
      const f4v t = L.tw1[k1 - 1][lane];
      z0[k1] = cmul_a(z0[k1], t.xy);
      z1[k1] = cmul_a(z1[k1], t.zw);
    }
#endif
  };
  const int k1 = lane >> 3, a0 = lane & 7, hh = lane & 7;
  auto r_mid = [&](c2 (&u)[16]) __attribute__((always_inline)) {
#ifndef XK_NORANGEFFT
    dft16p<1>(u);
#pragma unroll
    for (int s1 = 1; s1 < 16; s1 += 2) {
      const f4v t = L.tw2[s1 >> 1][lane];
      u[s1] = cmul_a(u[s1], t.xy);
      if (s1 < 15) u[s1 + 1] = cmul_a(u[s1 + 1], t.zw);
    }
#endif
  };
  auto r_t2 = [&](const c2 (&u)[16], c2 (&q0)[8], c2 (&q1)[8]) __attribute__((always_inline)) {
#pragma unroll
    for (int h = 0; h < 8; ++h)
      *reinterpret_cast<f4v*>(&rt[lane * 18 + 2 * h]) = f4v{u[2 * h].x, u[2 * h].y, u[2 * h + 1].x, u[2 * h + 1].y};
    cfence();
#pragma unroll
    for (int jj = 0; jj < 8; ++jj) {
      const f4v t = *reinterpret_cast<const f4v*>(&rt[(k1 * 8 + jj) * 18 + 2 * hh]);
      q0[jj] = t.xy;
      q1[jj] = t.zw;
    }
    cfence();
  };
  auto r_end = [&](c2 (&q0)[8], c2 (&q1)[8], char* __restrict__ slot) __attribute__((always_inline)) {
#ifndef XK_NORANGEFFT
    dft8p(q0);
    dft8p(q1);
#endif
    const int c = k * NW + w;
    const __amdgpu_buffer_rsrc_t rs = __builtin_amdgcn_make_buffer_rsrc(slot, (short)0, kSlotBytes, 0x00020000);
    const bool odd = lane & 1;
    const int gl = (lane >> 5) + (odd ? 2 : 0), el = c * GP + (lane & 31) - (odd ? 1 : 0);
#pragma unroll
    for (int s2 = 0; s2 < 8; ++s2) {
      const f4v v = pair_cols(q0[s2], q1[s2], odd);
      const int gb = (4 * s2 + gl) * C * GP * 8;
      if (H && ((s16m >> s2) & 1)) {
        const __half2 h0 = __floats2half2_rn(v.x * kXS, v.y * kXS), h1 = __floats2half2_rn(v.z * kXS, v.w * kXS);
        __builtin_amdgcn_raw_buffer_store_b64(u2v{__builtin_bit_cast(unsigned, h0), __builtin_bit_cast(unsigned, h1)}, rs,
                                              gb + el * 4, 0, 0);
      } else {
        __builtin_amdgcn_raw_buffer_store_b128(v, rs, gb + el * 8, 0, 0);
      }
    }
  };

#else
#ifdef XK_NOREF
#error "the half-frame build keeps the reference chirp"
#endif
  const int eh = w >> 2;
  const bool refw0 = k == 0 && (w & 3) == 0;
  typedef _Float16 h2v __attribute__((ext_vector_type(2)));
  using XH = std::conditional_t<H, h2v, c2>;
  auto ld_chirp_h = [&](int64_t f, int hf, XH (&xin)[8]) __attribute__((always_inline)) {
    const XH* __restrict__ q = reinterpret_cast<const XH*>(iq + (f * C + (128 * hf + 4 * k + (w & 3))) * (int64_t)S2) + eh;
#pragma unroll
    for (int i = 0; i < 8; ++i) {
      const int p = lane + 64 * i;
      if constexpr (FULL) xin[i] = __builtin_nontemporal_load(q + 2 * p);
      else xin[i] = __builtin_nontemporal_load(q + 2 * (p < S2 ? p : 0));
    }
  };
  auto rh_sum = [&](const XH (&xin)[8], bool refw, int xb, c2 (&d)[8]) __attribute__((always_inline)) {
    const float dsc = refw ? 0.f : 1.f;
    const c2* x0p = reinterpret_cast<const c2*>(L.x0[xb]) + eh;
    c2 sm{0.f, 0.f};
#pragma unroll
    for (int i = 0; i < 8; ++i) {
      c2 t;
      if constexpr (H) t = __builtin_convertvector(xin[i], c2);
      else t = xin[i];
      t = __builtin_elementwise_fma(c2{-dsc, -dsc}, x0p[2 * (lane + 64 * i)], t);
      if constexpr (!FULL)
        if (!(lane + 64 * i < S2)) t = c2{0.f, 0.f};
      d[i] = t;
      sm += t;
    }
    sm = wave_sum_c(sm);
    if (lane == 0) L.psum[w] = sm;
  };
  auto rh_prep = [&](c2 (&z)[8], bool refw) __attribute__((always_inline)) {
    const c2 csum_w = refw ? csum : c2{0.f, 0.f};
    const c2 mu = (L.psum[w] + L.psum[w ^ 4] - csum_w) * invS;
    float wv[8];
#pragma unroll
    for (int g = 0; g < 4; ++g) {
      const f4v t = L.wq[g][lane];
      wv[2 * g] = eh ? t.y : t.x;
      wv[2 * g + 1] = eh ? t.w : t.z;
    }
    if (refw) {
#pragma unroll
      for (int i = 0; i < 8; ++i) z[i] = __builtin_elementwise_fma(z[i] - mu, c2{wv[i], wv[i]}, -L.cwq[2 * i + eh][lane]);
    } else {
#pragma unroll
      for (int i = 0; i < 8; ++i) z[i] = (z[i] - mu) * wv[i];
    }
    dft8p(z);
#pragma unroll
    for (int k1 = 1; k1 < 8; ++k1) z[k1] = cmul_a(z[k1], L.th1[k1 - 1][lane]);
  };
  auto rh_t1w = [&](const c2 (&z)[8]) __attribute__((always_inline)) {
#pragma unroll
    for (int k1 = 0; k1 < 8; ++k1) rt[k1 * 72 + lane] = z[k1];
    cfence();
  };
  auto rh_t1r = [&](c2 (&u)[8]) __attribute__((always_inline)) {
#pragma unroll
    for (int l1 = 0; l1 < 8; ++l1) u[l1] = rt[(lane >> 3) * 72 + (lane & 7) + 8 * l1];
    cfence();
  };
  auto rh_mid = [&](c2 (&u)[8], c2 (&v)[8]) __attribute__((always_inline)) {
    dft8p(u);
#pragma unroll
    for (int s1 = 1; s1 < 8; ++s1) u[s1] = cmul_a(u[s1], L.th2[s1 - 1][lane]);
#pragma unroll
    for (int s1 = 0; s1 < 8; ++s1) rt[s1 * 97 + lane + 4 * (lane >> 5)] = u[s1];
    cfence();
    const int rb = (lane >> 3) * 97 + 8 * (lane & 7) + 4 * ((lane & 7) >> 2);
#pragma unroll
    for (int l0 = 0; l0 < 8; ++l0) v[l0] = rt[rb + l0];
    cfence();
    dft8p(v);
#pragma unroll
    for (int s2 = 0; s2 < 8; ++s2) rt[s2 * 64 + lane] = v[s2];
  };
  auto rh_end = [&](c2 (&v)[8], char* __restrict__ slot) __attribute__((always_inline)) {
    const c2* pr = L.u.rt[w ^ 4];
    if (eh) {
#pragma unroll
      for (int s2 = 0; s2 < 8; ++s2) v[s2] = pr[s2 * 64 + lane] - cmul_a(v[s2], L.thc[s2][lane]);
    } else {
#pragma unroll
      for (int s2 = 0; s2 < 8; ++s2) v[s2] = v[s2] + cmul_a(pr[s2 * 64 + lane], L.thc[s2][lane]);
    }
    constexpr int64_t kHalfBytes = (int64_t)NK * (C / 2) * GP * kES;
    const __amdgpu_buffer_rsrc_t rs = __builtin_amdgcn_make_buffer_rsrc(slot, (short)0, kHalfBytes, 0x00020000);
    const bool odd = lane & 1;
    const int ch = 4 * k + (w & 3);
    const int gl = (lane >> 5) + (odd ? 2 : 0), el = ch * GP + (lane & 31) - (odd ? 1 : 0);
#pragma unroll
    for (int t = 0; t < 4; ++t) {
      const f4v pv = pair_cols(v[2 * t], v[2 * t + 1], odd);
      const int gb = (16 * eh + 4 * t + gl) * (C / 2) * GP * 8;
      if (H && ((s16m >> (4 * eh + t)) & 1)) {
        const __half2 h0 = __floats2half2_rn(pv.x * kXS, pv.y * kXS), h1 = __floats2half2_rn(pv.z * kXS, pv.w * kXS);
        __builtin_amdgcn_raw_buffer_store_b64(u2v{__builtin_bit_cast(unsigned, h0), __builtin_bit_cast(unsigned, h1)}, rs,
                                              gb + el * 4, 0, 0);
      } else {
        __builtin_amdgcn_raw_buffer_store_b128(pv, rs, gb + el * 8, 0, 0);
      }
    }
  };
#endif

  auto ld_group = [&](const char* __restrict__ grp, f4v (&t)[8], auto G16) __attribute__((always_inline)) {
    constexpr int NL = decltype(G16)::value ? 4 : 8;
    const __amdgpu_buffer_rsrc_t rs = __builtin_amdgcn_make_buffer_rsrc(const_cast<char*>(grp), (short)0, C * GP * kES, 0x00020000);
#pragma unroll
    for (int i = 0; i < NL; ++i) t[i] = __builtin_amdgcn_raw_buffer_load_b128(rs, (tid + 512 * i) * 16, 0, 16);
  };
  auto stage = [&](const f4v (&t)[8], auto G16) __attribute__((always_inline)) {
    if constexpr (decltype(G16)::value) {
#pragma unroll
      for (int i = 0; i < 4; ++i) {
        const int e = tid + 512 * i;
        const u4v u = __builtin_bit_cast(u4v, t[i]);
        f4v* d = &L.u.stg[(e >> 3) * 17 + (e & 7) * 2];
        const bool sw = (e >> 2) & 1;
#ifndef XK_ST16SEL
        const float2 b0 = h2f(sw ? u.z : u.x), b1 = h2f(sw ? u.w : u.y), c0 = h2f(sw ? u.x : u.z), c1 = h2f(sw ? u.y : u.w);
        d[sw ? 1 : 0] = f4v{b0.x, b0.y, b1.x, b1.y};
        d[sw ? 0 : 1] = f4v{c0.x, c0.y, c1.x, c1.y};
#else
        const float2 a0 = h2f(u.x), a1 = h2f(u.y), a2 = h2f(u.z), a3 = h2f(u.w);
        const f4v lo = f4v{a0.x, a0.y, a1.x, a1.y}, hi = f4v{a2.x, a2.y, a3.x, a3.y};
        d[sw ? 1 : 0] = sw ? hi : lo;
        d[sw ? 0 : 1] = sw ? lo : hi;
#endif
      }
    } else {
#pragma unroll
      for (int i = 0; i < 8; ++i) {
        const int e4 = tid + 512 * i;
        L.u.stg[(e4 >> 4) * 17 + (e4 & 15)] = t[i];
      }
    }
  };
  const int pp = lane >> 4, q = lane & 15, p = 4 * w + pp;
  const int r = xcd_bin(k, p);
  auto d_rows = [&](int64_t f, c2 (&xv)[16], c2& x0r, c2& mu, auto G16) __attribute__((always_inline)) {
    {
      const c2* stg = reinterpret_cast<const c2*>(L.u.stg);
#pragma unroll
      for (int i = 0; i < 16; ++i) xv[i] = stg[(q + 16 * i) * 34 + p];
    }
#ifndef XK_NOREF
    x0r = reinterpret_cast<const c2*>(L.u.stg)[p];
    if (q == 0) xv[0] = c2{0.f, 0.f};
    float pm = fmaxf(fmaxf(abs2v(xv[0] + x0r), abs2v(xv[1] + x0r)), fmaxf(abs2v(xv[2] + x0r), abs2v(xv[3] + x0r)));
#pragma unroll
    for (int i = 4; i < 16; i += 4)
      pm = fmaxf(pm, fmaxf(fmaxf(abs2v(xv[i] + x0r), abs2v(xv[i + 1] + x0r)),
                           fmaxf(abs2v(xv[i + 2] + x0r), abs2v(xv[i + 3] + x0r))));
    c2 sm = (xv[0] + xv[1]) + (xv[2] + xv[3]);
#pragma unroll
    for (int i = 4; i < 16; i += 4) sm += (xv[i] + xv[i + 1]) + (xv[i + 2] + xv[i + 3]);
#else
    x0r = c2{0.f, 0.f};
    c2 sm = (xv[0] + xv[1]) + (xv[2] + xv[3]);
    float pm = fmaxf(fmaxf(abs2v(xv[0]), abs2v(xv[1])), fmaxf(abs2v(xv[2]), abs2v(xv[3])));
#pragma unroll
    for (int i = 4; i < 16; i += 4) {
      sm += (xv[i] + xv[i + 1]) + (xv[i + 2] + xv[i + 3]);
      pm = fmaxf(pm, fmaxf(fmaxf(abs2v(xv[i]), abs2v(xv[i + 1])), fmaxf(abs2v(xv[i + 2]), abs2v(xv[i + 3]))));
    }
#endif
    sm = c2{row_sum16(sm.x), row_sum16(sm.y)};
    pm = __int_as_float(row_max16(__float_as_int(pm)));
    mu = sm * (1.0f / (float)C);
    const float pr = decltype(G16)::value ? sqrtf(pm) * kXU : sqrtf(pm);
    a.profile[f * NR + r] = pr;
    if (q == 0) {
      const double rng = (double)r * a.dist_per_bin;
      L.key[p] = (r >= 1 && r <= NR - 2 && rng >= a.min_d && rng <= a.max_d && pr > a.range_thr) ? pr : -1.f;
    }
  };
  auto d_cand = [&](int64_t f, const c2 (&xv)[16], c2 x0r, auto G16) __attribute__((always_inline)) {
    float kv = lane < GP ? L.key[lane] : -1.f;
    const int ki = xcd_bin(k, lane & (GP - 1));
#pragma unroll
    for (int c = 0; c < XCD_CAND; ++c) {
      float bv = kv;
      int bi = ki;
      wave_argmax_dpp(bv, bi);
      const int sel = (bv < 0.f || a.force_fix) ? -1 : bi;
      if (w == 0 && lane == 0) a.cand_idx[(f * XCD_TILES + k) * XCD_CAND + c] = sel;
      if (sel >= 0 && r == sel) {
        float* __restrict__ row = a.cand_rows + ((f * XCD_TILES + k) * XCD_CAND + c) * (int64_t)C;
#pragma unroll
        for (int i = 0; i < 16; ++i) {
          const float v = abs2v(xv[i] + x0r);
          row[q + 16 * i] = decltype(G16)::value ? v * (kXU * kXU) : v;
        }
      }
      if (ki == sel) kv = -1.f;
    }
  };
  auto d_a = [&](c2 (&xv)[16], c2 mu) __attribute__((always_inline)) {
#pragma unroll
    for (int i = 0; i < 16; ++i) xv[i] = xv[i] - mu;
    c2 s2 = (xv[0] + xv[1]) + (xv[2] + xv[3]);
#pragma unroll
    for (int i = 4; i < 16; i += 4) s2 += (xv[i] + xv[i + 1]) + (xv[i + 2] + xv[i + 3]);
    mu = c2{row_sum16(s2.x), row_sum16(s2.y)} * (1.0f / (float)C);
#pragma unroll
    for (int g = 0; g < 4; ++g) {
      const f4v wv = L.wdl[g][lane];
      xv[4 * g + 0] = (xv[4 * g + 0] - mu) * wv.x;
      xv[4 * g + 1] = (xv[4 * g + 1] - mu) * wv.y;
      xv[4 * g + 2] = (xv[4 * g + 2] - mu) * wv.z;
      xv[4 * g + 3] = (xv[4 * g + 3] - mu) * wv.w;
    }
#ifndef XK_NODOPFFT
    dft16p<1>(xv);
#pragma unroll
    for (int d0 = 1; d0 < 16; d0 += 2) {
      const f4v t = L.twd[d0 >> 1][lane];
      xv[d0] = cmul_a(xv[d0], t.xy);
      if (d0 < 15) xv[d0 + 1] = cmul_a(xv[d0 + 1], t.zw);
    }
#endif
  };
  auto d_td = [&](c2 (&xv)[16]) __attribute__((always_inline)) {
#pragma unroll
    for (int h = 0; h < 8; ++h)
      *reinterpret_cast<f4v*>(&rt[304 * pp + 18 * q + 2 * h]) = f4v{xv[2 * h].x, xv[2 * h].y, xv[2 * h + 1].x, xv[2 * h + 1].y};
    cfence();
#pragma unroll
    for (int m0 = 0; m0 < 16; ++m0) xv[m0] = rt[304 * pp + 18 * m0 + q];
    cfence();
  };
  auto d_store = [&](int64_t f, const c2 (&xv)[16]) __attribute__((always_inline)) {
    if constexpr (RD) {
      const __amdgpu_buffer_rsrc_t rr = __builtin_amdgcn_make_buffer_rsrc(
          static_cast<char*>(a.rd) + f * NR * (int64_t)C * (H ? 4 : 8), (short)0, NR * C * (H ? 4 : 8), 0x00020000);
#pragma unroll
      for (int d1s = 0; d1s < 16; ++d1s) {
        const int off = r * C + q + 16 * d1s;
        if constexpr (H) {
          const c2 o = xv[(d1s + 8) & 15];
          __builtin_amdgcn_raw_buffer_store_b32(__builtin_bit_cast(unsigned, __floats2half2_rn(o.x, o.y)), rr, off * 4, 0,
                                                kRdAux);
        } else {
          __builtin_amdgcn_raw_buffer_store_b64(__builtin_bit_cast(u2v, xv[(d1s + 8) & 15]), rr, off * 8, 0, kRdAux);
        }
      }
    } else {
      float m = abs2v(xv[8]);
#pragma unroll
      for (int d1s = 1; d1s < 16; ++d1s) m = fmaxf(m, abs2v(xv[(d1s + 8) & 15]));
      const float rm = __int_as_float(row_max16(__float_as_int(m)));
      int e = INT_MAX;
#pragma unroll
      for (int d1s = 15; d1s >= 0; --d1s)
        if (abs2v(xv[(d1s + 8) & 15]) == rm) e = q + 16 * d1s;
      e = row_min16(e);
      a.rowpk[f * NR + r] = make_int2(__float_as_int(sqrtf(rm)), e);
    }
  };

  char* __restrict__ slots0 = reinterpret_cast<char*>(a.xcube) + (int64_t)x * NS * kSlotBytes;
#ifdef XK_DONE
  auto slot = [&](int) __attribute__((always_inline)) { return slots0; };
#else
  auto slot = [&](int j) __attribute__((always_inline)) { return slots0 + (int64_t)(j % kNS) * kSlotBytes; };
#endif
  auto frame = [&](int j) __attribute__((always_inline)) { return x + (int64_t)T * j; };
#ifndef XK_HALF
  TP xin[8];
#else
  XH xin[8];
#endif
  f4v grp[8];
#ifndef XK_HALF
  if (nj > 0) ld_chirp(frame(0), xin);
#else
  if (nj > 0) ld_chirp_h(frame(0), 0, xin);
#endif
#ifndef XK_HALF
  constexpr int kRDs = RD ? 16 : 1;
  auto body = [&](int j, auto DJ, auto RJ, auto PUB, auto CNT, auto GJ, auto NEXT, auto G16) __attribute__((always_inline)) {
    const bool dj = DJ, rj = RJ, pub = PUB, gj = GJ, next = NEXT;
    const int64_t fd = frame(j - 1 - kLag);
    if (j >= 1) __syncthreads();
    stamp(0);
#ifndef XK_NOREF
    if (rj)
      if (j >= 1) put_ref(0);
#endif
    if (dj) stage(grp, G16);
    stamp(1);
    if constexpr (std::is_same_v<decltype(PUB), bool>) vm_wait<0>();
    else if (pub) vm_wait<decltype(CNT)::value>();
    __syncthreads();
    if (pub)
      if (lane == 0)
        __hip_atomic_fetch_add(w == 0 ? rdy((j - 1) % kNS) : a.xctr + XCD_IDLE + (x * NK + k) * 32 + w,
                               w == 0 ? 1u : 0u, __ATOMIC_RELAXED, __HIP_MEMORY_SCOPE_AGENT);
#ifdef XK_SKEW
    if (pub && w == 0 && lane == 0 && j < XK_SKEW_STEPS)
      a.dbg[(int64_t)(x * NK + k) * (2 * XK_SKEW_STEPS) + 2 * j] = __builtin_amdgcn_s_memrealtime();
#endif
    stamp(2);
    c2 z0[8], z1[8], u[16];
    c2 xv[16], x0r{0.f, 0.f}, dmu{0.f, 0.f};
    if (dj) d_rows(fd, xv, x0r, dmu, G16);
    stamp(3);
    if (dj) __syncthreads();
    stamp(4);
    if (dj) d_cand(fd, xv, x0r, G16);
    stamp(5);
#define XK_POLL()                                                                                                   \
  do {                                                                                                              \
    wait_ge(rdy((j - kLag) % kNS), (unsigned)(NK * ((j - kLag) / kNS + 1)), a.xctr + XCD_ABORT, a.xerr);   \
    if (lane == 0) __hip_atomic_store(&gflag, (unsigned)j, __ATOMIC_RELAXED, __HIP_MEMORY_SCOPE_WORKGROUP);         \
  } while (0)
    if (XK_POLLAT == 1 && gj && w == 0) XK_POLL();
    if (rj) r_prep(xin, z0, z1);
    if (next) {
      const int jn = j + 1 < nj ? j + 1 : nj - 1;
#ifndef XK_NOREF
      ld_ref(frame(jn));
#endif
      ld_chirp(frame(jn), xin);
    }
    if (XK_POLLAT == 2 && gj && w == 0) XK_POLL();
#ifdef XK_SKEW
    if (gj && w == 0 && lane == 0 && j < XK_SKEW_STEPS)
      a.dbg[(int64_t)(x * NK + k) * (2 * XK_SKEW_STEPS) + 2 * j + 1] = __builtin_amdgcn_s_memrealtime();
#endif
    if (dj) d_a(xv, dmu);
    stamp(6);
    if (gj) {
      if (w == 0) {
        XK_POLL();
      } else {
        while (*reinterpret_cast<volatile unsigned*>(&gflag) < (unsigned)j) __builtin_amdgcn_s_sleep(1);
      }
      ld_group(slot(j - kLag) + (int64_t)k * C * GP * kES, grp, G16);
    }
    stamp(7);
#ifndef XK_NODOPFFT
    if (dj) d_td(xv);
#endif
    if (rj) {
#pragma unroll
      for (int kk = 0; kk < 8; ++kk)
        *reinterpret_cast<f4v*>(&rt[kk * 136 + 2 * lane]) = f4v{z0[kk].x, z0[kk].y, z1[kk].x, z1[kk].y};
      cfence();
    }
#ifndef XK_NODOPFFT
    if (dj) dft16p<1>(xv);
#endif
    if (rj) {
#pragma unroll
      for (int a1 = 0; a1 < 16; ++a1) u[a1] = rt[k1 * 136 + a0 + 8 * a1];
      cfence();
    }
    if (rj) {
      c2 q0[8], q1[8];
      r_mid(u);
      r_t2(u, q0, q1);
#ifdef XK_DONE
      static_assert(kLag == 1, "the done-counter A/B is written for lag 1");
      if (gj) {
        vm_wait<0>();
        __syncthreads();
        if (w == 0) {
          if (lane == 0) __hip_atomic_fetch_add(done, 1u, __ATOMIC_RELAXED, __HIP_MEMORY_SCOPE_AGENT);
          wait_ge(done, (unsigned)(NK * j), a.xctr + XCD_ABORT, a.xerr);
        }
        __syncthreads();
      }
#endif
      r_end(q0, q1, slot(j));
    }
    stamp(8);
    if (dj) d_store(fd, xv);
    stamp(9);
  };
  using T_ = std::true_type;
  using F_ = std::false_type;
  using C0 = std::integral_constant<int, 0>;
  using C1 = std::integral_constant<int, 0>;
  using CF = std::integral_constant<int, kRDs>;
  auto run = [&](auto G16) __attribute__((always_inline)) {
#if XK_LAG == 2
    if (nj >= 5) {
      body(0,      F_{}, T_{}, F_{}, C0{},                          F_{}, T_{}, G16);
      body(1,      F_{}, T_{}, T_{}, C0{},                          F_{}, T_{}, G16);
      body(2,      F_{}, T_{}, T_{}, C0{},                          T_{}, T_{}, G16);
      body(3,      T_{}, T_{}, T_{}, C0{},                          T_{}, T_{}, G16);
      for (int j = 4; j < nj; ++j) body(j, T_{}, T_{}, T_{}, CF{}, T_{}, T_{}, G16);
      body(nj,     T_{}, F_{}, T_{}, CF{},                          T_{}, F_{}, G16);
      body(nj + 1, T_{}, F_{}, F_{}, C0{},                          T_{}, F_{}, G16);
      body(nj + 2, T_{}, F_{}, F_{}, C0{},                          F_{}, F_{}, G16);
    } else {
      for (int j = 0; j < nj + 3; ++j)
        body(j, j >= 3, j < nj, j >= 1 && j - 1 < nj, C0{}, j >= 2 && j - 2 < nj, j + 1 < nj, G16);
    }
    return;
#endif
    if (FULL && nj >= 3) {
      body(0,      F_{}, T_{}, F_{}, C0{},                          F_{}, T_{}, G16);
      body(1,      F_{}, T_{}, T_{}, C1{},                          T_{}, T_{}, G16);
      body(2,      T_{}, T_{}, T_{}, C1{},                          T_{}, T_{}, G16);
      for (int j = 3; j < nj; ++j) body(j, T_{}, T_{}, T_{}, CF{}, T_{}, T_{}, G16);
      body(nj,     T_{}, F_{}, T_{}, CF{},                          T_{}, F_{}, G16);
      body(nj + 1, T_{}, F_{}, F_{}, C0{},                          F_{}, F_{}, G16);
    } else {
      for (int j = 0; j < nj + 2; ++j)
        body(j, j >= 2, j < nj, j >= 1 && j - 1 < nj, C0{}, j >= 1 && j - 1 < nj, j + 1 < nj, G16);
    }
  };
  if constexpr (H) {
    if (g16) run(T_{});
    else run(F_{});
  } else {
    run(F_{});
  }
#else
  (void)ld_chirp;
  (void)ld_group;
  (void)slot;
  (void)stamp;
  constexpr int64_t kHalfSlot = (int64_t)NK * (C / 2) * GP * kES;
  auto hslot = [&](int h) __attribute__((always_inline)) { return slots0 + (int64_t)(h % kNS) * kHalfSlot; };
  constexpr int kRDs = RD ? 16 : 1;
  const int nh = 2 * nj;
  c2 xvd[16];
  auto ld_group_h = [&](int hh, auto HFL, auto G16) __attribute__((always_inline)) {
    constexpr int NL = decltype(G16)::value ? 2 : 4;
    const char* grb = hslot(hh) + (int64_t)k * (C / 2) * GP * kES;
    const __amdgpu_buffer_rsrc_t rs = __builtin_amdgcn_make_buffer_rsrc(const_cast<char*>(grb), (short)0, (C / 2) * GP * kES, 0x00020000);
    if constexpr (std::is_same_v<decltype(HFL), bool>) {
#pragma unroll
      for (int i = 0; i < NL; ++i) {
        const f4v t = __builtin_amdgcn_raw_buffer_load_b128(rs, (tid + 512 * i) * 16, 0, 16);
        grp[i] = HFL ? grp[i] : t;
        grp[NL + i] = HFL ? t : grp[NL + i];
      }
    } else {
#pragma unroll
      for (int i = 0; i < NL; ++i)
        grp[decltype(HFL)::value * NL + i] = __builtin_amdgcn_raw_buffer_load_b128(rs, (tid + 512 * i) * 16, 0, 16);
    }
  };
  typedef __attribute__((address_space(3))) unsigned lu32;
  lu32* const gfl = (lu32*)&gflag;
#define XK_HPOLL()                                                                                                  \
  do {                                                                                                              \
    wait_ge(rdy((h - kLag) % kNS), (unsigned)(NK * ((h - kLag) / kNS + 1)), a.xctr + XCD_ABORT, a.xerr);   \
    if (lane == 0) __hip_atomic_store(gfl, (unsigned)h, __ATOMIC_RELAXED, __HIP_MEMORY_SCOPE_WORKGROUP);             \
  } while (0)
  auto hbody = [&](int h, auto D1, auto D2, auto RJ, auto PUB, auto CNT, auto GJ, auto NEXT, auto HF, auto GHF,
                   auto G16) __attribute__((always_inline)) {
    const bool d1 = D1, d2 = D2, rj = RJ, pub = PUB, gj = GJ, next = NEXT;
    const bool hf = HF;
    const int64_t fd1 = frame((h - 2 - kLag) >> 1), fd2 = frame((h - 3 - kLag) >> 1);
    if (h >= 1) __syncthreads();
    if (hf && h + 1 < nh) put_ref(((h + 1) >> 1) & 1);
    if (d1) stage(grp, G16);
    c2 z[8], u[8];
    if (rj) rh_sum(xin, refw0 && !hf, (h >> 1) & 1, z);
    if constexpr (std::is_same_v<decltype(PUB), bool>) vm_wait<0>();
    else if (pub) vm_wait<decltype(CNT)::value>();
    __syncthreads();
    if (pub)
      if (lane == 0)
        __hip_atomic_fetch_add(w == 0 ? rdy((h - 1) % kNS) : a.xctr + XCD_IDLE + (x * NK + k) * 32 + w,
                               w == 0 ? 1u : 0u, __ATOMIC_RELAXED, __HIP_MEMORY_SCOPE_AGENT);
    c2 x0r{0.f, 0.f}, dmu{0.f, 0.f};
    if (d1) d_rows(fd1, xvd, x0r, dmu, G16);
    if (d1) __syncthreads();
    if (d1) d_cand(fd1, xvd, x0r, G16);
    if (rj) rh_prep(z, refw0 && !hf);
    if (next) {
      const int hn = h + 1;
      if (!hf && h + 2 < nh) ld_ref(frame((h >> 1) + 1));
      ld_chirp_h(frame(hn >> 1), hn & 1, xin);
    }
    if (XK_POLLAT == 2 && gj && w == 0) XK_HPOLL();
    if (d1) d_a(xvd, dmu);
    if (gj) {
      if (w == 0) {
        XK_HPOLL();
      } else {
        while (__hip_atomic_load(gfl, __ATOMIC_RELAXED, __HIP_MEMORY_SCOPE_WORKGROUP) < (unsigned)h) __builtin_amdgcn_s_sleep(1);
      }
      ld_group_h(h - kLag, GHF, G16);
    }
    if (d2) d_td(xvd);
    if (rj) rh_t1w(z);
    if (d2) dft16p<1>(xvd);
    if (rj) {
      rh_t1r(u);
      rh_mid(u, z);
    }
    __syncthreads();
    if (rj) rh_end(z, hslot(h));
    if (d2) d_store(fd2, xvd);
  };
#undef XK_HPOLL
  using T_ = std::true_type;
  using F_ = std::false_type;
  using C0 = std::integral_constant<int, 0>;
  constexpr int P0 = kLag == 1 ? 4 : 6;
  const int nhs = nh + 2 + kLag;
  auto pro = [&](auto HC, auto G16) __attribute__((always_inline)) {
    constexpr int h = decltype(HC)::value;
    hbody(h, std::bool_constant<(h >= 2 + kLag && ((h - 2 - kLag) & 1) == 0)>{},
          std::bool_constant<(h >= 3 + kLag && ((h - 3 - kLag) & 1) == 0)>{}, T_{}, std::bool_constant<(h >= 1)>{},
          std::integral_constant<int, (h - 1 >= 3 + kLag && ((h - 4 - kLag) & 1) == 0) ? kRDs : 0>{},
          std::bool_constant<(h >= kLag)>{}, T_{}, std::bool_constant<(h & 1) != 0>{},
          std::bool_constant<(((h - kLag) & 1) != 0)>{}, G16);
  };
  auto mid = [&](int h, auto G16) __attribute__((always_inline)) {
    constexpr bool d1o = kLag & 1;
    hbody(h, std::bool_constant<!d1o>{}, std::bool_constant<d1o>{}, T_{}, T_{},
          std::integral_constant<int, d1o ? 0 : kRDs>{}, T_{}, T_{}, F_{}, std::bool_constant<(kLag & 1) != 0>{}, G16);
    hbody(h + 1, std::bool_constant<d1o>{}, std::bool_constant<!d1o>{}, T_{}, T_{},
          std::integral_constant<int, d1o ? kRDs : 0>{}, T_{}, T_{}, T_{}, std::bool_constant<(kLag & 1) == 0>{}, G16);
  };
  auto epi = [&](auto IC, auto G16) __attribute__((always_inline)) {
    constexpr int i = decltype(IC)::value;
    hbody(nh - 2 + i, std::bool_constant<((kLag + i) & 1) == 0 && i < 4 + kLag>{},
          std::bool_constant<((kLag + i + 1) & 1) == 0 && i < 5 + kLag>{}, std::bool_constant<(i < 2)>{},
          std::bool_constant<(i < 3)>{}, std::integral_constant<int, ((kLag + i) & 1) == 0 ? kRDs : 0>{},
          std::bool_constant<(i < 2 + kLag)>{}, std::bool_constant<(i == 0)>{}, std::bool_constant<(i & 1) != 0>{},
          std::bool_constant<((i + kLag) & 1) != 0>{}, G16);
  };
  auto hrun = [&](auto G16) __attribute__((always_inline)) {
    if (nh - 2 > P0) {
      using std::integral_constant;
      pro(integral_constant<int, 0>{}, G16);
      pro(integral_constant<int, 1>{}, G16);
      pro(integral_constant<int, 2>{}, G16);
      pro(integral_constant<int, 3>{}, G16);
      if constexpr (P0 > 4) {
        pro(integral_constant<int, 4>{}, G16);
        pro(integral_constant<int, 5>{}, G16);
      }
      for (int h = P0; h < nh - 2; h += 2) mid(h, G16);
      epi(integral_constant<int, 0>{}, G16);
      epi(integral_constant<int, 1>{}, G16);
      epi(integral_constant<int, 2>{}, G16);
      epi(integral_constant<int, 3>{}, G16);
      epi(integral_constant<int, 4>{}, G16);
      if constexpr (kLag == 2) epi(integral_constant<int, 5>{}, G16);
    } else {
      for (int h = 0; h < nhs; ++h) {
        const int h1 = h - 2 - kLag, h2 = h - 3 - kLag;
        hbody(h, h1 >= 0 && !(h1 & 1) && (h1 >> 1) < nj, h2 >= 0 && !(h2 & 1) && (h2 >> 1) < nj, h < nh,
              h >= 1 && h - 1 < nh, C0{}, h >= kLag && h - kLag < nh, h + 1 < nh, (h & 1) != 0, ((h - kLag) & 1) != 0, G16);
      }
    }
  };
  if constexpr (H) {
    if (g16) hrun(T_{});
    else hrun(F_{});
  } else {
    hrun(F_{});
  }
#endif
  if (stamper) {
    a.clk[2] = __builtin_amdgcn_s_memtime();
    a.clk[3] = __builtin_amdgcn_s_memrealtime();
  }
#ifdef XK_STAMPS
  if (lane == 0 && (w == 0 || w == 4)) {
    unsigned long long* d = a.dbg + ((int64_t)blockIdx.x * 2 + (w >> 2)) * 16;
    for (int i = 0; i < NST; ++i) d[i] = st_acc[i];
    d[13] = __builtin_amdgcn_s_memtime() - st_c0;
    d[14] = __builtin_amdgcn_s_memrealtime() - st_r0;
    d[15] = (unsigned long long)nj;
  }
#endif
}

__global__ __launch_bounds__(512, 1) void k_xcd_census(int* out) {
  if (threadIdx.x == 0) {
    unsigned xcc;
    asm volatile("s_getreg_b32 %0, hwreg(HW_REG_XCC_ID)" : "=s"(xcc));
    out[blockIdx.x] = (int)(xcc & 15);
  }
}

namespace {
std::mutex xcd_chain_mu;
hipEvent_t xcd_chain_ev[64] = {};
}

hipError_t launch_xcd(const OnePassArgs& a, hipStream_t s) {
  if (a.F <= 0) return hipSuccess;
  if (!onepass_supported(a.S, a.C, op::NR, a.C) || a.slots < 4 || a.slots > XCD_MAX_SLOTS) return hipErrorInvalidValue;
  int dev = 0;
  hipError_t e = hipGetDevice(&dev);
  if (e != hipSuccess) return e;
  if (dev < 0 || dev >= 64) return hipErrorInvalidDevice;
  std::lock_guard<std::mutex> lk(xcd_chain_mu);
  if (!xcd_chain_ev[dev]) {
    if ((e = hipEventCreateWithFlags(&xcd_chain_ev[dev], hipEventDisableTiming | kEvDevice)) != hipSuccess) return e;
  } else if (hipStreamWaitEvent(s, xcd_chain_ev[dev], 0) != hipSuccess) {
    (void)hipGetLastError();
    if ((e = hipEventCreateWithFlags(&xcd_chain_ev[dev], hipEventDisableTiming | kEvDevice)) != hipSuccess) return e;
  }
  if (!a.xclr || a.xmemset)
    if ((e = hipMemsetAsync(a.xctr, 0, sizeof(unsigned) * XCD_CTR_WORDS, s)) != hipSuccess) return e;
  if (a.nteams < 1 || a.nteams > 8) return hipErrorInvalidValue;
  const dim3 g(xk::NK * a.nteams), bl(64 * xk::NW);
  const char* coop_env = std::getenv("FMCW_XCD_COOP");
  const bool coop = coop_env && coop_env[0] == '1';
  auto go = [&](auto kern) {
    if (!coop) {
      hipLaunchKernelGGL(kern, g, bl, 0, s, a);
      return hipGetLastError();
    }
    void* args[] = {const_cast<OnePassArgs*>(&a)};
    return hipLaunchCooperativeKernel(reinterpret_cast<const void*>(kern), g, bl, args, 0, s);
  };
  const bool rd = a.rd != nullptr;
  if (a.S == op::NR) {
    if (a.h) e = rd ? go(k_rdx<true, true, true>) : go(k_rdx<true, true, false>);
    else e = rd ? go(k_rdx<true, false, true>) : go(k_rdx<true, false, false>);
  } else {
    if (a.h) e = rd ? go(k_rdx<false, true, true>) : go(k_rdx<false, true, false>);
    else e = rd ? go(k_rdx<false, false, true>) : go(k_rdx<false, false, false>);
  }
  if (e != hipSuccess) {
    (void)hipGetLastError();
    return e;
  }
  return hipEventRecord(xcd_chain_ev[dev], s);
}

hipError_t xcd_census(int* nteams, int8_t* xcc_team) {
  *nteams = 0;
  for (int i = 0; i < 16; ++i) xcc_team[i] = -1;
  int dev = 0, cus = 0;
  hipError_t e = hipGetDevice(&dev);
  if (e == hipSuccess) e = hipDeviceGetAttribute(&cus, hipDeviceAttributeMultiprocessorCount, dev);
  if (e != hipSuccess) return e;
  const bool dbg = [] { const char* v = std::getenv("FMCW_XCD_DEBUG"); return v && v[0] == '1'; }();
  if (cus < xk::NK || cus > XCD_GRID || cus % xk::NK) {
    if (dbg) std::fprintf(stderr, "xcd_census: %d CUs\n", cus);
    return hipSuccess;
  }
  {
    const void* ks[] = {reinterpret_cast<const void*>(k_rdx<true, false, true>), reinterpret_cast<const void*>(k_rdx<true, false, false>),
                        reinterpret_cast<const void*>(k_rdx<true, true, true>), reinterpret_cast<const void*>(k_rdx<true, true, false>),
                        reinterpret_cast<const void*>(k_rdx<false, false, true>), reinterpret_cast<const void*>(k_rdx<false, false, false>),
                        reinterpret_cast<const void*>(k_rdx<false, true, true>), reinterpret_cast<const void*>(k_rdx<false, true, false>)};
    for (const void* kf : ks) {
      int nb = 0;
      if ((e = hipOccupancyMaxActiveBlocksPerMultiprocessor(&nb, kf, 64 * xk::NW, 0)) != hipSuccess) return e;
      if (nb < 1) {
        if (dbg) std::fprintf(stderr, "xcd_census: k_rdx not resident at one block per CU\n");
        return hipSuccess;
      }
    }
  }
  int* d = nullptr;
  if ((e = hipMalloc(&d, XCD_GRID * sizeof(int))) != hipSuccess) return e;
  int h[XCD_GRID];
  hipLaunchKernelGGL(k_xcd_census, dim3(cus), dim3(512), sizeof(xk::LdsX), 0, d);
  e = hipGetLastError();
  if (e == hipSuccess) e = hipMemcpy(h, d, sizeof(int) * cus, hipMemcpyDeviceToHost);
  (void)hipFree(d);
  if (e != hipSuccess) return e;
  int n[16] = {};
  bool good = true;
  for (int b = 0; b < cus; ++b) {
    if (h[b] < 0 || h[b] > 15) good = false;
    else ++n[h[b]];
  }
  int t = 0;
  for (int i = 0; i < 16 && good; ++i) {
    if (n[i] == 0) continue;
    if (n[i] != xk::NK) good = false;
    else xcc_team[i] = (int8_t)t++;
  }
  good = good && t * xk::NK == cus;
  if (good) *nteams = t;
  else
    for (int i = 0; i < 16; ++i) xcc_team[i] = -1;
  if (dbg) {
    std::fprintf(stderr, "xcd_census: cus %d teams %d, XCC of blocks 0..15:", cus, *nteams);
    for (int b = 0; b < 16 && b < cus; ++b) std::fprintf(stderr, " %d", h[b]);
    std::fprintf(stderr, "\n");
  }
  return hipSuccess;
}

}
```

Baseline: 920,600.

## Reuse one cube slot per team by alternating transposed placement between frames

New measurement: 980,900, median of 6. 1.07x the previous value.

```diff
diff --git a/fmcw_radar_processing_amd/csrc/fmcw_api.cpp b/fmcw_radar_processing_amd/csrc/fmcw_api.cpp
--- a/fmcw_radar_processing_amd/csrc/fmcw_api.cpp
+++ b/fmcw_radar_processing_amd/csrc/fmcw_api.cpp
@@ -459,9 +459,6 @@
       for (int e = 0; e < 2; ++e) xput(fmcw::XT_R1 + (2 * (k1 - 1) + e) * 64 + l, (2 * l + e) * k1);
     for (int s1 = 1; s1 < 16; ++s1) xput(fmcw::XT_R2 + (s1 - 1) * 64 + l, 8 * ((l & 7) * s1));
     for (int d0 = 1; d0 < 16; ++d0) xput(fmcw::XT_D1 + (d0 - 1) * 64 + l, 4 * ((l & 15) * d0));
-    for (int k1 = 1; k1 < 8; ++k1) xput(fmcw::XT_H1 + (k1 - 1) * 64 + l, 2 * l * k1);
-    for (int s1 = 1; s1 < 8; ++s1) xput(fmcw::XT_H2 + (s1 - 1) * 64 + l, 16 * ((l & 7) * s1));
-    for (int s2 = 0; s2 < 8; ++s2) xput(fmcw::XT_HC + s2 * 64 + l, l + 64 * s2);
   }
   CHK(c->x_tab.ensure(xt.size() * 4));
   HIPCHK(hipMemcpyAsync(c->x_tab.p, xt.data(), xt.size() * 4, hipMemcpyHostToDevice, s));
@@ -499,7 +496,7 @@
   const int64_t chunk = std::min<int64_t>(F, c->chunk_frames > 0 ? c->chunk_frames : 8192);
   const int tiles = fmcw::XCD_TILES, ncand = fmcw::XCD_CAND;
   const int TC = tiles * ncand;
-  const int slots = fmcw::XCD_MAX_SLOTS;
+  const int slots = 1;
   {
 #ifdef FMCW_XCUBE_PAD_AB
     CHK(c->x_cube.ensure((size_t)8 * slots * fmcw::XCD_TILES * C * 32 * 8 + ((size_t)1 << 30)));
diff --git a/fmcw_radar_processing_amd/csrc/fmcw_internal.h b/fmcw_radar_processing_amd/csrc/fmcw_internal.h
--- a/fmcw_radar_processing_amd/csrc/fmcw_internal.h
+++ b/fmcw_radar_processing_amd/csrc/fmcw_internal.h
@@ -1,6 +1,8 @@
 #pragma once
 #include <hip/hip_runtime.h>
 #include <stdint.h>
+
+#include "xcd_place.h"
 
 namespace fmcw {
 
@@ -111,21 +113,12 @@
 constexpr int XT_R1 = 0;
 constexpr int XT_R2 = 14 * 64;
 constexpr int XT_D1 = 29 * 64;
-constexpr int XT_H1 = 44 * 64;
-constexpr int XT_H2 = 51 * 64;
-constexpr int XT_HC = 58 * 64;
-constexpr int XT_SIZE = 66 * 64;
-#ifndef XK_HALF
+constexpr int XT_SIZE = 44 * 64;
 __host__ __device__ inline int xcd_bin(int g, int p) {
   return (p >> 3) + 4 * (g & 1) + 8 * ((g >> 1) & 1) + 16 * (p & 7) + 128 * (g >> 2);
 }
 __host__ __device__ inline int xcd_group(int r) { return ((r >> 2) & 1) | (((r >> 3) & 1) << 1) | ((r >> 7) << 2); }
 __host__ __device__ inline int xcd_pos(int r) { return ((r & 3) << 3) | ((r >> 4) & 7); }
-#else
-__host__ __device__ inline int xcd_bin(int g, int p) { return 32 * g + p; }
-__host__ __device__ inline int xcd_group(int r) { return r >> 5; }
-__host__ __device__ inline int xcd_pos(int r) { return r & 31; }
-#endif
 
 struct Detect1pArgs {
   const float* profile;
diff --git a/fmcw_radar_processing_amd/csrc/kernels_xcd.hip b/fmcw_radar_processing_amd/csrc/kernels_xcd.hip
--- a/fmcw_radar_processing_amd/csrc/kernels_xcd.hip
+++ b/fmcw_radar_processing_amd/csrc/kernels_xcd.hip
@@ -17,22 +17,15 @@
 #define XK_RD_AUX 2
 #endif
 constexpr int kRdAux = XK_RD_AUX;
-#ifndef XK_LAG
-#define XK_LAG 1
-#endif
-#ifndef XK_NS
-#define XK_NS (2 * XK_LAG)
-#endif
-constexpr int kLag = XK_LAG;
+constexpr int kLag = 1;
 #ifndef XK_POLLAT
 #define XK_POLLAT 2
 #endif
 #ifndef XK_SKEW_STEPS
 #define XK_SKEW_STEPS 256
 #endif
-static_assert(kLag == 1 || kLag == 2, "poll lag 1 (shipped) or 2");
-constexpr int kNS = XK_NS;
-static_assert(kNS >= 2 * kLag && kNS <= 4, "slot reuse: seeing ready(j - lag) proves frame j - 2 lag read");
+constexpr int kNS = 2;
+static_assert(kNS >= 2 && kNS <= XCD_MAX_SLOTS, "a counter is reused only after every member has seen its last value");
 constexpr int NK = 32;
 constexpr int C = 256;
 constexpr int NW = 8;
@@ -40,32 +33,26 @@
 typedef unsigned u2v __attribute__((ext_vector_type(2)));
 typedef unsigned u4v __attribute__((ext_vector_type(4)));
 static_assert(NK * NW == C && NK * GP == NR && NK == XCD_TILES, "team geometry");
+static_assert(NK * NK * XCD_PLACE_BYTES == NK * C * GP * 8 && NW * XCD_ROW_BYTES == XCD_PLACE_BYTES && GP * 8 == XCD_ROW_BYTES,
+              "the slot is 32 x 32 places of 8 rows");
+static_assert(xcd_place(0, 3, 5) == 3 * xcd_place(0, 1, 0) + 5 * xcd_place(0, 0, 1) &&
+              xcd_place(1, 3, 5) == 3 * xcd_place(1, 1, 0) + 5 * xcd_place(1, 0, 1) && xcd_place(0, 0, 0) == 0 && xcd_place(1, 0, 0) == 0,
+              "k_rdx addresses a place by two strides");
 
 struct LdsX {
   union {
     f4v stg[C * 17];
     c2 rt[NW][1216];
   } u;
-#ifndef XK_HALF
   f4v tw1[7][64];
   f4v tw2[8][64];
-#else
-  c2 th1[7][64];
-  c2 th2[7][64];
-  c2 thc[8][64];
-#endif
   f4v twd[8][64];
   f4v wdl[4][64];
   f4v wq[4][64];
   c2 cwq[16][64];
   float key[GP];
 #ifndef XK_NOREF
-#ifndef XK_HALF
   f4v x0[512];
-#else
-  f4v x0[2][512];
-  c2 psum[8];
-#endif
 #endif
 };
 
@@ -166,9 +153,6 @@
   const int S = FULL ? NR : a.S, S2 = S >> 1, NS = a.slots;
   unsigned* ready = a.xctr + (x * 2 + 0) * 32 * XCD_MAX_SLOTS;
   auto rdy = [&](int s_) __attribute__((always_inline)) -> unsigned* { return &ready[s_ * 32]; };
-#ifdef XK_DONE
-  unsigned* done = ready + 32 * XCD_MAX_SLOTS;
-#endif
 
   using TP = std::conditional_t<H, h4v, f4v>;
   const TP* __restrict__ iq = reinterpret_cast<const TP*>(a.iq);
@@ -190,16 +174,11 @@
     else t = x0n;
     if constexpr (!FULL)
       if (tid >= S2) t = f4v{0.f, 0.f, 0.f, 0.f};
-#ifndef XK_HALF
     (void)b;
     L.x0[tid] = t;
-#else
-    L.x0[b][tid] = t;
-#endif
   };
   if (nj > 0) ld_ref(x);
 #endif
-#ifndef XK_HALF
   for (int i = tid; i < 44 * 64; i += 512) {
     const c2 v = tov(a.xtab[i]);
     const int l = i & 63;
@@ -209,19 +188,6 @@
     else { const int t = (i - XT_D1) >> 6; d = reinterpret_cast<c2*>(&L.twd[t >> 1][l]) + (t & 1); }
     *d = v;
   }
-#else
-  for (int i = XT_D1 + tid; i < XT_H1; i += 512) {
-    const int t = (i - XT_D1) >> 6;
-    reinterpret_cast<c2*>(&L.twd[t >> 1][i & 63])[t & 1] = tov(a.xtab[i]);
-  }
-  for (int i = tid; i < 22 * 64; i += 512) {
-    const c2 v = tov(a.xtab[XT_H1 + i]);
-    const int t = i >> 6, l = i & 63;
-    if (t < 7) L.th1[t][l] = v;
-    else if (t < 14) L.th2[t - 7][l] = v;
-    else L.thc[t - 14][l] = v;
-  }
-#endif
   const float wd_scale = (H && RD ? a.rd_scale : 1.0f) * (g16 ? kXU : 1.0f);
   for (int i = tid; i < 16 * 64; i += 512)
     reinterpret_cast<float*>(&L.wdl[i >> 8][i & 63])[(i >> 6) & 3] = a.wd[(i & 15) + 16 * (i >> 6)] * wd_scale;
@@ -265,7 +231,6 @@
   };
 
   c2* const rt = L.u.rt[w];
-#ifndef XK_HALF
 #ifndef XK_NOREF
   const bool refw = k == 0 && w == 0;
   const float dsc = refw ? 0.f : 1.f;
@@ -347,152 +312,48 @@
     }
     cfence();
   };
-  auto r_end = [&](c2 (&q0)[8], c2 (&q1)[8], char* __restrict__ slot) __attribute__((always_inline)) {
+  auto r_end = [&](c2 (&q0)[8], c2 (&q1)[8], char* __restrict__ slot, int j) __attribute__((always_inline)) {
 #ifndef XK_NORANGEFFT
     dft8p(q0);
     dft8p(q1);
 #endif
-    const int c = k * NW + w;
     const __amdgpu_buffer_rsrc_t rs = __builtin_amdgcn_make_buffer_rsrc(slot, (short)0, kSlotBytes, 0x00020000);
     const bool odd = lane & 1;
-    const int gl = (lane >> 5) + (odd ? 2 : 0), el = c * GP + (lane & 31) - (odd ? 1 : 0);
+    const int gl = (lane >> 5) + (odd ? 2 : 0), pl = (lane & 31) - (odd ? 1 : 0);
+    vm_wait<0>();
+    const int sg = xcd_place(j, 1, 0) * XCD_PLACE_BYTES, sk = xcd_place(j, 0, 1) * XCD_PLACE_BYTES;
+    const int vb = gl * sg + k * sk + w * XCD_ROW_BYTES;
 #pragma unroll
     for (int s2 = 0; s2 < 8; ++s2) {
       const f4v v = pair_cols(q0[s2], q1[s2], odd);
-      const int gb = (4 * s2 + gl) * C * GP * 8;
       if (H && ((s16m >> s2) & 1)) {
         const __half2 h0 = __floats2half2_rn(v.x * kXS, v.y * kXS), h1 = __floats2half2_rn(v.z * kXS, v.w * kXS);
         __builtin_amdgcn_raw_buffer_store_b64(u2v{__builtin_bit_cast(unsigned, h0), __builtin_bit_cast(unsigned, h1)}, rs,
-                                              gb + el * 4, 0, 0);
+                                              vb + pl * 4 + 4 * s2 * sg, 0, 0);
       } else {
-        __builtin_amdgcn_raw_buffer_store_b128(v, rs, gb + el * 8, 0, 0);
+        __builtin_amdgcn_raw_buffer_store_b128(v, rs, vb + pl * 8 + 4 * s2 * sg, 0, 0);
       }
     }
   };
 
-#else
-#ifdef XK_NOREF
-#error "the half-frame build keeps the reference chirp"
-#endif
-  const int eh = w >> 2;
-  const bool refw0 = k == 0 && (w & 3) == 0;
-  typedef _Float16 h2v __attribute__((ext_vector_type(2)));
-  using XH = std::conditional_t<H, h2v, c2>;
-  auto ld_chirp_h = [&](int64_t f, int hf, XH (&xin)[8]) __attribute__((always_inline)) {
-    const XH* __restrict__ q = reinterpret_cast<const XH*>(iq + (f * C + (128 * hf + 4 * k + (w & 3))) * (int64_t)S2) + eh;
-#pragma unroll
-    for (int i = 0; i < 8; ++i) {
-      const int p = lane + 64 * i;
-      if constexpr (FULL) xin[i] = __builtin_nontemporal_load(q + 2 * p);
-      else xin[i] = __builtin_nontemporal_load(q + 2 * (p < S2 ? p : 0));
-    }
-  };
-  auto rh_sum = [&](const XH (&xin)[8], bool refw, int xb, c2 (&d)[8]) __attribute__((always_inline)) {
-    const float dsc = refw ? 0.f : 1.f;
-    const c2* x0p = reinterpret_cast<const c2*>(L.x0[xb]) + eh;
-    c2 sm{0.f, 0.f};
-#pragma unroll
-    for (int i = 0; i < 8; ++i) {
-      c2 t;
-      if constexpr (H) t = __builtin_convertvector(xin[i], c2);
-      else t = xin[i];
-      t = __builtin_elementwise_fma(c2{-dsc, -dsc}, x0p[2 * (lane + 64 * i)], t);
-      if constexpr (!FULL)
-        if (!(lane + 64 * i < S2)) t = c2{0.f, 0.f};
-      d[i] = t;
-      sm += t;
-    }
-    sm = wave_sum_c(sm);
-    if (lane == 0) L.psum[w] = sm;
-  };
-  auto rh_prep = [&](c2 (&z)[8], bool refw) __attribute__((always_inline)) {
-    const c2 csum_w = refw ? csum : c2{0.f, 0.f};
-    const c2 mu = (L.psum[w] + L.psum[w ^ 4] - csum_w) * invS;
-    float wv[8];
-#pragma unroll
-    for (int g = 0; g < 4; ++g) {
-      const f4v t = L.wq[g][lane];
-      wv[2 * g] = eh ? t.y : t.x;
-      wv[2 * g + 1] = eh ? t.w : t.z;
-    }
-    if (refw) {
-#pragma unroll
-      for (int i = 0; i < 8; ++i) z[i] = __builtin_elementwise_fma(z[i] - mu, c2{wv[i], wv[i]}, -L.cwq[2 * i + eh][lane]);
-    } else {
-#pragma unroll
-      for (int i = 0; i < 8; ++i) z[i] = (z[i] - mu) * wv[i];
-    }
-    dft8p(z);
-#pragma unroll
-    for (int k1 = 1; k1 < 8; ++k1) z[k1] = cmul_a(z[k1], L.th1[k1 - 1][lane]);
-  };
-  auto rh_t1w = [&](const c2 (&z)[8]) __attribute__((always_inline)) {
-#pragma unroll
-    for (int k1 = 0; k1 < 8; ++k1) rt[k1 * 72 + lane] = z[k1];
-    cfence();
-  };
-  auto rh_t1r = [&](c2 (&u)[8]) __attribute__((always_inline)) {
-#pragma unroll
-    for (int l1 = 0; l1 < 8; ++l1) u[l1] = rt[(lane >> 3) * 72 + (lane & 7) + 8 * l1];
-    cfence();
-  };
-  auto rh_mid = [&](c2 (&u)[8], c2 (&v)[8]) __attribute__((always_inline)) {
-    dft8p(u);
-#pragma unroll
-    for (int s1 = 1; s1 < 8; ++s1) u[s1] = cmul_a(u[s1], L.th2[s1 - 1][lane]);
-#pragma unroll
-    for (int s1 = 0; s1 < 8; ++s1) rt[s1 * 97 + lane + 4 * (lane >> 5)] = u[s1];
-    cfence();
-    const int rb = (lane >> 3) * 97 + 8 * (lane & 7) + 4 * ((lane & 7) >> 2);
-#pragma unroll
-    for (int l0 = 0; l0 < 8; ++l0) v[l0] = rt[rb + l0];
-    cfence();
-    dft8p(v);
-#pragma unroll
-    for (int s2 = 0; s2 < 8; ++s2) rt[s2 * 64 + lane] = v[s2];
-  };
-  auto rh_end = [&](c2 (&v)[8], char* __restrict__ slot) __attribute__((always_inline)) {
-    const c2* pr = L.u.rt[w ^ 4];
-    if (eh) {
-#pragma unroll
-      for (int s2 = 0; s2 < 8; ++s2) v[s2] = pr[s2 * 64 + lane] - cmul_a(v[s2], L.thc[s2][lane]);
-    } else {
-#pragma unroll
-      for (int s2 = 0; s2 < 8; ++s2) v[s2] = v[s2] + cmul_a(pr[s2 * 64 + lane], L.thc[s2][lane]);
-    }
-    constexpr int64_t kHalfBytes = (int64_t)NK * (C / 2) * GP * kES;
-    const __amdgpu_buffer_rsrc_t rs = __builtin_amdgcn_make_buffer_rsrc(slot, (short)0, kHalfBytes, 0x00020000);
-    const bool odd = lane & 1;
-    const int ch = 4 * k + (w & 3);
-    const int gl = (lane >> 5) + (odd ? 2 : 0), el = ch * GP + (lane & 31) - (odd ? 1 : 0);
-#pragma unroll
-    for (int t = 0; t < 4; ++t) {
-      const f4v pv = pair_cols(v[2 * t], v[2 * t + 1], odd);
-      const int gb = (16 * eh + 4 * t + gl) * (C / 2) * GP * 8;
-      if (H && ((s16m >> (4 * eh + t)) & 1)) {
-        const __half2 h0 = __floats2half2_rn(pv.x * kXS, pv.y * kXS), h1 = __floats2half2_rn(pv.z * kXS, pv.w * kXS);
-        __builtin_amdgcn_raw_buffer_store_b64(u2v{__builtin_bit_cast(unsigned, h0), __builtin_bit_cast(unsigned, h1)}, rs,
-                                              gb + el * 4, 0, 0);
-      } else {
-        __builtin_amdgcn_raw_buffer_store_b128(pv, rs, gb + el * 8, 0, 0);
-      }
-    }
-  };
-#endif
-
-  auto ld_group = [&](const char* __restrict__ grp, f4v (&t)[8], auto G16) __attribute__((always_inline)) {
-    constexpr int NL = decltype(G16)::value ? 4 : 8;
-    const __amdgpu_buffer_rsrc_t rs = __builtin_amdgcn_make_buffer_rsrc(const_cast<char*>(grp), (short)0, C * GP * kES, 0x00020000);
-#pragma unroll
-    for (int i = 0; i < NL; ++i) t[i] = __builtin_amdgcn_raw_buffer_load_b128(rs, (tid + 512 * i) * 16, 0, 16);
+
+  auto ld_group = [&](const char* __restrict__ slot, int j, f4v (&t)[8], auto G16) __attribute__((always_inline)) {
+    constexpr bool g16_ = decltype(G16)::value;
+    constexpr int NL = g16_ ? 4 : 8;
+    const __amdgpu_buffer_rsrc_t rs = __builtin_amdgcn_make_buffer_rsrc(const_cast<char*>(slot), (short)0, kSlotBytes, 0x00020000);
+    const int sk = xcd_place(j, 1, 0) * XCD_PLACE_BYTES, sm = xcd_place(j, 0, 1) * XCD_PLACE_BYTES;
+    const int vo = g16_ ? (lane >> 3) * sm + (lane & 7) * 16 : (lane >> 4) * sm + (lane & 15) * 16;
+    const int sb = k * sk + w * XCD_ROW_BYTES;
+#pragma unroll
+    for (int i = 0; i < NL; ++i) t[i] = __builtin_amdgcn_raw_buffer_load_b128(rs, vo, sb + (g16_ ? 8 : 4) * i * sm, 16);
   };
   auto stage = [&](const f4v (&t)[8], auto G16) __attribute__((always_inline)) {
     if constexpr (decltype(G16)::value) {
 #pragma unroll
       for (int i = 0; i < 4; ++i) {
-        const int e = tid + 512 * i;
+        const int e = lane & 7;
         const u4v u = __builtin_bit_cast(u4v, t[i]);
-        f4v* d = &L.u.stg[(e >> 3) * 17 + (e & 7) * 2];
+        f4v* d = &L.u.stg[(8 * (8 * i + (lane >> 3)) + w) * 17 + e * 2];
         const bool sw = (e >> 2) & 1;
 #ifndef XK_ST16SEL
         const float2 b0 = h2f(sw ? u.z : u.x), b1 = h2f(sw ? u.w : u.y), c0 = h2f(sw ? u.x : u.z), c1 = h2f(sw ? u.y : u.w);
@@ -507,10 +368,7 @@
       }
     } else {
 #pragma unroll
-      for (int i = 0; i < 8; ++i) {
-        const int e4 = tid + 512 * i;
-        L.u.stg[(e4 >> 4) * 17 + (e4 & 15)] = t[i];
-      }
+      for (int i = 0; i < 8; ++i) L.u.stg[(8 * (4 * i + (lane >> 4)) + w) * 17 + (lane & 15)] = t[i];
     }
   };
   const int pp = lane >> 4, q = lane & 15, p = 4 * w + pp;
@@ -636,25 +494,11 @@
     }
   };
 
-  char* __restrict__ slots0 = reinterpret_cast<char*>(a.xcube) + (int64_t)x * NS * kSlotBytes;
-#ifdef XK_DONE
-  auto slot = [&](int) __attribute__((always_inline)) { return slots0; };
-#else
-  auto slot = [&](int j) __attribute__((always_inline)) { return slots0 + (int64_t)(j % kNS) * kSlotBytes; };
-#endif
+  char* __restrict__ slot = reinterpret_cast<char*>(a.xcube) + (int64_t)x * NS * kSlotBytes;
   auto frame = [&](int j) __attribute__((always_inline)) { return x + (int64_t)T * j; };
-#ifndef XK_HALF
   TP xin[8];
-#else
-  XH xin[8];
-#endif
   f4v grp[8];
-#ifndef XK_HALF
   if (nj > 0) ld_chirp(frame(0), xin);
-#else
-  if (nj > 0) ld_chirp_h(frame(0), 0, xin);
-#endif
-#ifndef XK_HALF
   constexpr int kRDs = RD ? 16 : 1;
   auto body = [&](int j, auto DJ, auto RJ, auto PUB, auto CNT, auto GJ, auto NEXT, auto G16) __attribute__((always_inline)) {
     const bool dj = DJ, rj = RJ, pub = PUB, gj = GJ, next = NEXT;
@@ -714,7 +558,7 @@
       } else {
         while (*reinterpret_cast<volatile unsigned*>(&gflag) < (unsigned)j) __builtin_amdgcn_s_sleep(1);
       }
-      ld_group(slot(j - kLag) + (int64_t)k * C * GP * kES, grp, G16);
+      ld_group(slot, j - kLag, grp, G16);
     }
     stamp(7);
 #ifndef XK_NODOPFFT
@@ -738,19 +582,7 @@
       c2 q0[8], q1[8];
       r_mid(u);
       r_t2(u, q0, q1);
-#ifdef XK_DONE
-      static_assert(kLag == 1, "the done-counter A/B is written for lag 1");
-      if (gj) {
-        vm_wait<0>();
-        __syncthreads();
-        if (w == 0) {
-          if (lane == 0) __hip_atomic_fetch_add(done, 1u, __ATOMIC_RELAXED, __HIP_MEMORY_SCOPE_AGENT);
-          wait_ge(done, (unsigned)(NK * j), a.xctr + XCD_ABORT, a.xerr);
-        }
-        __syncthreads();
-      }
-#endif
-      r_end(q0, q1, slot(j));
+      r_end(q0, q1, slot, j);
     }
     stamp(8);
     if (dj) d_store(fd, xv);
@@ -762,22 +594,6 @@
   using C1 = std::integral_constant<int, 0>;
   using CF = std::integral_constant<int, kRDs>;
   auto run = [&](auto G16) __attribute__((always_inline)) {
-#if XK_LAG == 2
-    if (nj >= 5) {
-      body(0,      F_{}, T_{}, F_{}, C0{},                          F_{}, T_{}, G16);
-      body(1,      F_{}, T_{}, T_{}, C0{},                          F_{}, T_{}, G16);
-      body(2,      F_{}, T_{}, T_{}, C0{},                          T_{}, T_{}, G16);
-      body(3,      T_{}, T_{}, T_{}, C0{},                          T_{}, T_{}, G16);
-      for (int j = 4; j < nj; ++j) body(j, T_{}, T_{}, T_{}, CF{}, T_{}, T_{}, G16);
-      body(nj,     T_{}, F_{}, T_{}, CF{},                          T_{}, F_{}, G16);
-      body(nj + 1, T_{}, F_{}, F_{}, C0{},                          T_{}, F_{}, G16);
-      body(nj + 2, T_{}, F_{}, F_{}, C0{},                          F_{}, F_{}, G16);
-    } else {
-      for (int j = 0; j < nj + 3; ++j)
-        body(j, j >= 3, j < nj, j >= 1 && j - 1 < nj, C0{}, j >= 2 && j - 2 < nj, j + 1 < nj, G16);
-    }
-    return;
-#endif
     if (FULL && nj >= 3) {
       body(0,      F_{}, T_{}, F_{}, C0{},                          F_{}, T_{}, G16);
       body(1,      F_{}, T_{}, T_{}, C1{},                          T_{}, T_{}, G16);
@@ -796,150 +612,6 @@
   } else {
     run(F_{});
   }
-#else
-  (void)ld_chirp;
-  (void)ld_group;
-  (void)slot;
-  (void)stamp;
-  constexpr int64_t kHalfSlot = (int64_t)NK * (C / 2) * GP * kES;
-  auto hslot = [&](int h) __attribute__((always_inline)) { return slots0 + (int64_t)(h % kNS) * kHalfSlot; };
-  constexpr int kRDs = RD ? 16 : 1;
-  const int nh = 2 * nj;
-  c2 xvd[16];
-  auto ld_group_h = [&](int hh, auto HFL, auto G16) __attribute__((always_inline)) {
-    constexpr int NL = decltype(G16)::value ? 2 : 4;
-    const char* grb = hslot(hh) + (int64_t)k * (C / 2) * GP * kES;
-    const __amdgpu_buffer_rsrc_t rs = __builtin_amdgcn_make_buffer_rsrc(const_cast<char*>(grb), (short)0, (C / 2) * GP * kES, 0x00020000);
-    if constexpr (std::is_same_v<decltype(HFL), bool>) {
-#pragma unroll
-      for (int i = 0; i < NL; ++i) {
-        const f4v t = __builtin_amdgcn_raw_buffer_load_b128(rs, (tid + 512 * i) * 16, 0, 16);
-        grp[i] = HFL ? grp[i] : t;
-        grp[NL + i] = HFL ? t : grp[NL + i];
-      }
-    } else {
-#pragma unroll
-      for (int i = 0; i < NL; ++i)
-        grp[decltype(HFL)::value * NL + i] = __builtin_amdgcn_raw_buffer_load_b128(rs, (tid + 512 * i) * 16, 0, 16);
-    }
-  };
-  typedef __attribute__((address_space(3))) unsigned lu32;
-  lu32* const gfl = (lu32*)&gflag;
-#define XK_HPOLL()                                                                                                  \
-  do {                                                                                                              \
-    wait_ge(rdy((h - kLag) % kNS), (unsigned)(NK * ((h - kLag) / kNS + 1)), a.xctr + XCD_ABORT, a.xerr);   \
-    if (lane == 0) __hip_atomic_store(gfl, (unsigned)h, __ATOMIC_RELAXED, __HIP_MEMORY_SCOPE_WORKGROUP);             \
-  } while (0)
-  auto hbody = [&](int h, auto D1, auto D2, auto RJ, auto PUB, auto CNT, auto GJ, auto NEXT, auto HF, auto GHF,
-                   auto G16) __attribute__((always_inline)) {
-    const bool d1 = D1, d2 = D2, rj = RJ, pub = PUB, gj = GJ, next = NEXT;
-    const bool hf = HF;
-    const int64_t fd1 = frame((h - 2 - kLag) >> 1), fd2 = frame((h - 3 - kLag) >> 1);
-    if (h >= 1) __syncthreads();
-    if (hf && h + 1 < nh) put_ref(((h + 1) >> 1) & 1);
-    if (d1) stage(grp, G16);
-    c2 z[8], u[8];
-    if (rj) rh_sum(xin, refw0 && !hf, (h >> 1) & 1, z);
-    if constexpr (std::is_same_v<decltype(PUB), bool>) vm_wait<0>();
-    else if (pub) vm_wait<decltype(CNT)::value>();
-    __syncthreads();
-    if (pub)
-      if (lane == 0)
-        __hip_atomic_fetch_add(w == 0 ? rdy((h - 1) % kNS) : a.xctr + XCD_IDLE + (x * NK + k) * 32 + w,
-                               w == 0 ? 1u : 0u, __ATOMIC_RELAXED, __HIP_MEMORY_SCOPE_AGENT);
-    c2 x0r{0.f, 0.f}, dmu{0.f, 0.f};
-    if (d1) d_rows(fd1, xvd, x0r, dmu, G16);
-    if (d1) __syncthreads();
-    if (d1) d_cand(fd1, xvd, x0r, G16);
-    if (rj) rh_prep(z, refw0 && !hf);
-    if (next) {
-      const int hn = h + 1;
-      if (!hf && h + 2 < nh) ld_ref(frame((h >> 1) + 1));
-      ld_chirp_h(frame(hn >> 1), hn & 1, xin);
-    }
-    if (XK_POLLAT == 2 && gj && w == 0) XK_HPOLL();
-    if (d1) d_a(xvd, dmu);
-    if (gj) {
-      if (w == 0) {
-        XK_HPOLL();
-      } else {
-        while (__hip_atomic_load(gfl, __ATOMIC_RELAXED, __HIP_MEMORY_SCOPE_WORKGROUP) < (unsigned)h) __builtin_amdgcn_s_sleep(1);
-      }
-      ld_group_h(h - kLag, GHF, G16);
-    }
-    if (d2) d_td(xvd);
-    if (rj) rh_t1w(z);
-    if (d2) dft16p<1>(xvd);
-    if (rj) {
-      rh_t1r(u);
-      rh_mid(u, z);
-    }
-    __syncthreads();
-    if (rj) rh_end(z, hslot(h));
-    if (d2) d_store(fd2, xvd);
-  };
-#undef XK_HPOLL
-  using T_ = std::true_type;
-  using F_ = std::false_type;
-  using C0 = std::integral_constant<int, 0>;
-  constexpr int P0 = kLag == 1 ? 4 : 6;
-  const int nhs = nh + 2 + kLag;
-  auto pro = [&](auto HC, auto G16) __attribute__((always_inline)) {
-    constexpr int h = decltype(HC)::value;
-    hbody(h, std::bool_constant<(h >= 2 + kLag && ((h - 2 - kLag) & 1) == 0)>{},
-          std::bool_constant<(h >= 3 + kLag && ((h - 3 - kLag) & 1) == 0)>{}, T_{}, std::bool_constant<(h >= 1)>{},
-          std::integral_constant<int, (h - 1 >= 3 + kLag && ((h - 4 - kLag) & 1) == 0) ? kRDs : 0>{},
-          std::bool_constant<(h >= kLag)>{}, T_{}, std::bool_constant<(h & 1) != 0>{},
-          std::bool_constant<(((h - kLag) & 1) != 0)>{}, G16);
-  };
-  auto mid = [&](int h, auto G16) __attribute__((always_inline)) {
-    constexpr bool d1o = kLag & 1;
-    hbody(h, std::bool_constant<!d1o>{}, std::bool_constant<d1o>{}, T_{}, T_{},
-          std::integral_constant<int, d1o ? 0 : kRDs>{}, T_{}, T_{}, F_{}, std::bool_constant<(kLag & 1) != 0>{}, G16);
-    hbody(h + 1, std::bool_constant<d1o>{}, std::bool_constant<!d1o>{}, T_{}, T_{},
-          std::integral_constant<int, d1o ? kRDs : 0>{}, T_{}, T_{}, T_{}, std::bool_constant<(kLag & 1) == 0>{}, G16);
-  };
-  auto epi = [&](auto IC, auto G16) __attribute__((always_inline)) {
-    constexpr int i = decltype(IC)::value;
-    hbody(nh - 2 + i, std::bool_constant<((kLag + i) & 1) == 0 && i < 4 + kLag>{},
-          std::bool_constant<((kLag + i + 1) & 1) == 0 && i < 5 + kLag>{}, std::bool_constant<(i < 2)>{},
-          std::bool_constant<(i < 3)>{}, std::integral_constant<int, ((kLag + i) & 1) == 0 ? kRDs : 0>{},
-          std::bool_constant<(i < 2 + kLag)>{}, std::bool_constant<(i == 0)>{}, std::bool_constant<(i & 1) != 0>{},
-          std::bool_constant<((i + kLag) & 1) != 0>{}, G16);
-  };
-  auto hrun = [&](auto G16) __attribute__((always_inline)) {
-    if (nh - 2 > P0) {
-      using std::integral_constant;
-      pro(integral_constant<int, 0>{}, G16);
-      pro(integral_constant<int, 1>{}, G16);
-      pro(integral_constant<int, 2>{}, G16);
-      pro(integral_constant<int, 3>{}, G16);
-      if constexpr (P0 > 4) {
-        pro(integral_constant<int, 4>{}, G16);
-        pro(integral_constant<int, 5>{}, G16);
-      }
-      for (int h = P0; h < nh - 2; h += 2) mid(h, G16);
-      epi(integral_constant<int, 0>{}, G16);
-      epi(integral_constant<int, 1>{}, G16);
-      epi(integral_constant<int, 2>{}, G16);
-      epi(integral_constant<int, 3>{}, G16);
-      epi(integral_constant<int, 4>{}, G16);
-      if constexpr (kLag == 2) epi(integral_constant<int, 5>{}, G16);
-    } else {
-      for (int h = 0; h < nhs; ++h) {
-        const int h1 = h - 2 - kLag, h2 = h - 3 - kLag;
-        hbody(h, h1 >= 0 && !(h1 & 1) && (h1 >> 1) < nj, h2 >= 0 && !(h2 & 1) && (h2 >> 1) < nj, h < nh,
-              h >= 1 && h - 1 < nh, C0{}, h >= kLag && h - kLag < nh, h + 1 < nh, (h & 1) != 0, ((h - kLag) & 1) != 0, G16);
-      }
-    }
-  };
-  if constexpr (H) {
-    if (g16) hrun(T_{});
-    else hrun(F_{});
-  } else {
-    hrun(F_{});
-  }
-#endif
   if (stamper) {
     a.clk[2] = __builtin_amdgcn_s_memtime();
     a.clk[3] = __builtin_amdgcn_s_memrealtime();
@@ -970,7 +642,7 @@
 
 hipError_t launch_xcd(const OnePassArgs& a, hipStream_t s) {
   if (a.F <= 0) return hipSuccess;
-  if (!onepass_supported(a.S, a.C, op::NR, a.C) || a.slots < 4 || a.slots > XCD_MAX_SLOTS) return hipErrorInvalidValue;
+  if (!onepass_supported(a.S, a.C, op::NR, a.C) || a.slots < 1 || a.slots > XCD_MAX_SLOTS) return hipErrorInvalidValue;
   int dev = 0;
   hipError_t e = hipGetDevice(&dev);
   if (e != hipSuccess) return e;
diff --git a/fmcw_radar_processing_amd/csrc/xcd_place.h b/fmcw_radar_processing_amd/csrc/xcd_place.h
--- /dev/null
+++ b/fmcw_radar_processing_amd/csrc/xcd_place.h
@@ -0,0 +1,8 @@
+#pragma once
+
+namespace fmcw {
+
+constexpr int XCD_PLACE_BYTES = 2048, XCD_ROW_BYTES = 256;
+constexpr int xcd_place(int j, int r, int w) { return (j & 1) ? 32 * w + r : 32 * r + w; }
+
+}
```
